# Orca0917/fine-grained-emotional-control-of-tts

Hardware: AMD Instinct MI355X
Metric: train mel-frames/sec at B=32, 80-bin mel; 1/2/4/8 MI355X (higher is better)
Workload: dtype bf16; 1 GPU; FastSpeech2 train step (fwd+loss+bwd+allreduce+AdamW), B=32/GPU, T_phon_max=200, T_mel_max=977, D=384 F=1536 6+6 FFT layers, 80 mels; global_batch=32, seq_len=977, parallelism=dp1

## Files before the change

fine-grained-emotional-control-of-tts_amd/csrc/gemm.hip:

```cpp
#include <type_traits>

#include "fs2_cdna.h"
#include "fs2_launch.h"

#include <cstdlib>
#include <cstring>

namespace {

#ifdef FS2_EXPERIMENTS
#define XFLAGS(p) ((p).g4_flags)
#else
#define XFLAGS(p) 0
#endif

constexpr int BM = 128, BN = 128, NT = 256;
constexpr int TILE_BYTES = 128 * 128;

struct GemmP {
  int M, N, K, kvalid, mvalid, nvalid;
  const char* A; long lda; const char* B; long ldb;
  int conv_mode, conv_t, conv_kw, conv_c, conv_p;
  int conv_dil;
  char* C; long ldc; int c_fp32; int c_conv_kw;
  const float* bias; int relu;
  const char* gate; long ldg;
  const float* row_scale;
  const char* residual; long ldr;
  const float* row_scale_post;
  int accumulate; int split_k; int k_per_split;
  long split_stride;
  int g4_flags;
  int batch_div;
  long sA1, sA2, sB1, sB2, sC1, sC2, sR1, sR2;
  int tiles_m, tiles_n;
  int vec_ok;
  int vec_align;
  int c_row_t, c_row_pad;
  int max_ctas;
  int a_bytes, b_bytes;
  int a_kw;
  const int32_t* k_eff;
};

__device__ __forceinline__ u32x4 add_bf16x8(u32x4 a, u32x4 b) {
  u32x4 r;
#pragma unroll
  for (int w = 0; w < 4; ++w) {
    float a0 = __builtin_bit_cast(float, a[w] << 16), a1 = __builtin_bit_cast(float, a[w] & 0xffff0000u);
    float b0 = __builtin_bit_cast(float, b[w] << 16), b1 = __builtin_bit_cast(float, b[w] & 0xffff0000u);
    bf16 r0 = (bf16)(a0 + b0), r1 = (bf16)(a1 + b1);
    r[w] = (unsigned)__builtin_bit_cast(unsigned short, r0) |
           ((unsigned)__builtin_bit_cast(unsigned short, r1) << 16);
  }
  return r;
}
__device__ __forceinline__ u32x4 add_f32x4(u32x4 a, u32x4 b) {
  const f32x4 fa = __builtin_bit_cast(f32x4, a), fb = __builtin_bit_cast(f32x4, b);
  return __builtin_bit_cast(u32x4, fa + fb);
}

__device__ __attribute__((noinline)) float epi_act_rare(float v, int act) {
  if (act == 2) return 0.5f * v * (1.f + erff(v * 0.70710678118654752f));
  if (act == 3) return v >= 0.f ? v : 0.1f * v;
  if (act == 4) return tanhf(v);
  return v;
}
__device__ __forceinline__ float epi_act(float v, int act) {
  if (act > 1) return epi_act_rare(v, act);
  return act ? fmaxf(v, 0.f) : v;
}

template <typename T>
struct Cfg {
  static constexpr int ES = sizeof(T);
  static constexpr int EPC = 16 / ES;
  static constexpr int BK = 8 * EPC;
};

__device__ __forceinline__ u32x4 ld16(const char* p) { return *(const u32x4*)p; }

template <typename T>
__device__ __forceinline__ void load_kmajor(u32x4 (&st)[4], const char* base, long ld, int row0,
                                            int nrows, int k0, int kend, const GemmP& p,
                                            int cmode, const int (&rb)[4], const int (&rt)[4]) {
  constexpr int ES = Cfg<T>::ES, EPC = Cfg<T>::EPC;
  const int tid = threadIdx.x;
  const int kc = tid & 7;
  const int k = k0 + kc * EPC;
#pragma unroll
  for (int i = 0; i < 4; ++i) {
    const int r = (tid >> 3) + 32 * i;
    const int row = row0 + r;
    u32x4 v = {0u, 0u, 0u, 0u};
    if (row < nrows && k < kend) {
      if (cmode == 0) {
        v = ld16(base + ((long)row * ld + k) * ES);
      } else {
        const int C = p.conv_c, T_ = p.conv_t, P = p.conv_p;
        const int j = k / C, c = k - j * C;
        const int b = rb[i], t = rt[i];
        if (cmode == 1) {
          const int ts = reflect_idx(t + (j - P) * p.conv_dil, T_);
          v = ld16(base + ((long)(b * T_ + ts) * ld + c) * ES);
        } else if (cmode == 5) {
          const int ts = t + (j - P) * p.conv_dil;
          if (ts >= 0 && ts < T_) v = ld16(base + ((long)(b * T_ + ts) * ld + c) * ES);
        } else if (cmode == 4) {
          const int ts = t - j;
          if (ts >= 0 && ts < T_) v = ld16(base + ((long)(b * T_ + ts) * ld + c) * ES);
        } else {
          const int t1 = t - j + P;
          if (t1 >= 0 && t1 < T_) v = ld16(base + ((long)(b * T_ + t1) * ld + c) * ES);
          const int t2 = P - j - t;
          if (t >= 1 && t2 >= 0 && t2 < T_) {
            u32x4 w = ld16(base + ((long)(b * T_ + t2) * ld + c) * ES);
            v = (ES == 2) ? add_bf16x8(v, w) : add_f32x4(v, w);
          }
          const int t3 = 2 * (T_ - 1) - t - j + P;
          if (t <= T_ - 2 && t3 >= 0 && t3 < T_ && t3 + j - P >= T_) {
            u32x4 w = ld16(base + ((long)(b * T_ + t3) * ld + c) * ES);
            v = (ES == 2) ? add_bf16x8(v, w) : add_f32x4(v, w);
          }
        }
      }
    }
// ... 153 lines not shown
  const int k1 = s * 32 + 8 * g + q, k2 = k1 + 4;
  const char* a1 = lds + k1 * ROWB + ((c ^ mn_swz<bf16>(k1)) << 4) + boff;
  const char* a2 = lds + k2 * ROWB + ((c ^ mn_swz<bf16>(k2)) << 4) + boff;
  s16x4 lo, hi;
  asm volatile("ds_read_b64_tr_b16 %0, %1" : "=v"(lo) : "v"(lds_off(a1)));
  asm volatile("ds_read_b64_tr_b16 %0, %1" : "=v"(hi) : "v"(lds_off(a2)));
  const s16x8 v = {lo[0], lo[1], lo[2], lo[3], hi[0], hi[1], hi[2], hi[3]};
  return __builtin_bit_cast(bf16x8, v);
}
__device__ __forceinline__ void mn_ready(bf16x8& f) { asm volatile("" : "+v"(f)); }

__device__ __forceinline__ float frag_f32_kmajor(const char* lds, int r0, int s, int lane) {
  const int r = r0 + (lane & 15);
  return *(const float*)(lds + r * 128 + ((s ^ (r & 7)) << 4) + (lane >> 4) * 4);
}
__device__ __forceinline__ float frag_f32_mnmajor(const char* lds, int r0, int s, int lane) {
  const int m = r0 + (lane & 15), k = s * 4 + (lane >> 4);
  return *(const float*)(lds + k * 512 + (((m >> 2) ^ mn_swz<float>(k)) << 4) + (m & 3) * 4);
}

template <typename T>
__device__ __forceinline__ void load8(float (&o)[8], const T* src, int nn) {
  if (nn == 8) {
    if constexpr (sizeof(T) == 2) {
      const u32x4 u = *(const u32x4*)src;
#pragma unroll
      for (int w = 0; w < 4; ++w) {
        o[2 * w] = __builtin_bit_cast(float, u[w] << 16);
        o[2 * w + 1] = __builtin_bit_cast(float, u[w] & 0xffff0000u);
      }
    } else {
      const f32x4 a = *(const f32x4*)src, b = *(const f32x4*)(src + 4);
      o[0] = a[0]; o[1] = a[1]; o[2] = a[2]; o[3] = a[3];
      o[4] = b[0]; o[5] = b[1]; o[6] = b[2]; o[7] = b[3];
    }
  } else {
    for (int e = 0; e < 8; ++e) o[e] = e < nn ? to_f(src[e]) : 0.f;
  }
}
template <typename T>
__device__ __forceinline__ void store8(T* dst, const float (&v)[8], int nn) {
  if (nn == 8) {
    if constexpr (sizeof(T) == 2) {
      u32x4 u;
#pragma unroll
      for (int w = 0; w < 4; ++w) {
        const bf16 a = (bf16)v[2 * w], b = (bf16)v[2 * w + 1];
        u[w] = (unsigned)__builtin_bit_cast(unsigned short, a) |
               ((unsigned)__builtin_bit_cast(unsigned short, b) << 16);
      }
      *(u32x4*)dst = u;
    } else {
      *(f32x4*)dst = f32x4{v[0], v[1], v[2], v[3]};
      *(f32x4*)(dst + 4) = f32x4{v[4], v[5], v[6], v[7]};
    }
  } else {
    for (int e = 0; e < nn; ++e) dst[e] = from_f<T>(v[e]);
  }
}

template <typename T, bool AK, bool BKM, bool GA, bool GB>
__global__ void __launch_bounds__(NT) gemm_kernel(GemmP p) {
  constexpr int ES = Cfg<T>::ES, BK = Cfg<T>::BK;
  __shared__ __attribute__((aligned(16))) char smem[2 * 2 * TILE_BYTES];

  const int tid = threadIdx.x, lane = tid & 63, wave = tid >> 6;
  const int wm = wave >> 1, wn = wave & 1;

  const int bid = blockIdx.x;
  const int tm = bid / p.tiles_n, tn = bid - tm * p.tiles_n;
  const int m0 = tm * BM, n0 = tn * BN;

  int z = 0, kbeg = 0, kend = p.K;
  if (p.split_k > 1) {
    kbeg = blockIdx.z * p.k_per_split;
    kend = min(p.K, kbeg + p.k_per_split);
  } else {
    z = blockIdx.z;
  }
  const long zb = z / p.batch_div, zh = z - zb * p.batch_div;
  const char* Ab = p.A + (zb * p.sA1 + zh * p.sA2) * ES;
  const char* Bb = p.B + (zb * p.sB1 + zh * p.sB2) * ES;
  const int kvalid = p.kvalid;

  int rb[4] = {0, 0, 0, 0}, rt[4] = {0, 0, 0, 0};
  const int amode = (p.conv_mode == 1 || p.conv_mode == 2 || p.conv_mode == 4 || p.conv_mode == 5) ? p.conv_mode : 0;
  if (AK && amode) {
#pragma unroll
    for (int i = 0; i < 4; ++i) {
      const int row = m0 + (GA ? (wave * 4 + i) * 8 + (lane >> 3) : (tid >> 3) + 32 * i);
      const int rpu = amode == 4 ? p.conv_t + 2 * p.conv_p : p.conv_t;
      rb[i] = row / rpu;
      rt[i] = row - rb[i] * rpu;
    }
  }
  const bool bconv3 = (p.conv_mode == 3);
  const int zero4[4] = {0, 0, 0, 0};

  f32x4 acc[4][4];
#pragma unroll
  for (int i = 0; i < 4; ++i)
#pragma unroll
    for (int j = 0; j < 4; ++j) acc[i][j] = f32x4{0.f, 0.f, 0.f, 0.f};

  u32x4 stA[4], stB[4];
  auto load_tiles = [&](int k0, int stage) {
    char* la = smem + stage * 2 * TILE_BYTES;
    char* lb = la + TILE_BYTES;
    const int wv = __builtin_amdgcn_readfirstlane(wave);
    if constexpr (GA) {
      if constexpr (AK) glds_kmajor(la, Ab, p.lda, m0, p.M, k0, kend, p, amode, rb, rt, wv, lane);
      else glds_mnmajor(la, Ab, p.lda, m0, p.M, k0, min(kend, kvalid), p, false, wv, lane);
    } else {
      if constexpr (AK) load_kmajor<T>(stA, Ab, p.lda, m0, p.M, k0, kend, p, amode, rb, rt);
      else load_mnmajor<T>(stA, Ab, p.lda, m0, p.M, k0, min(kend, kvalid), p, false);
    }
    if constexpr (GB) {
      if constexpr (BKM) glds_kmajor(lb, Bb, p.ldb, n0, p.N, k0, kend, p, 0, zero4, zero4, wv, lane);
      else glds_mnmajor(lb, Bb, p.ldb, n0, p.N, k0, min(kend, kvalid), p, bconv3, wv, lane);
    } else {
      if constexpr (BKM) load_kmajor<T>(stB, Bb, p.ldb, n0, p.N, k0, kend, p, 0, zero4, zero4);
      else load_mnmajor<T>(stB, Bb, p.ldb, n0, p.N, k0, min(kend, kvalid), p, bconv3);
    }
  };
  auto store_tiles = [&](int stage) {
    char* la = smem + stage * 2 * TILE_BYTES;
    char* lb = la + TILE_BYTES;
    if constexpr (!GA) { if constexpr (AK) store_kmajor<T>(la, stA); else store_mnmajor<T>(la, stA); }
    if constexpr (!GB) { if constexpr (BKM) store_kmajor<T>(lb, stB); else store_mnmajor<T>(lb, stB); }
  };

  const int nk = (kend > kbeg) ? (kend - kbeg + BK - 1) / BK : 0;
  if (nk > 0) {
    load_tiles(kbeg, 0);
    store_tiles(0);
  }
  __syncthreads();

  for (int kt = 0; kt < nk; ++kt) {
    const int stage = kt & 1;
    if (kt + 1 < nk) load_tiles(kbeg + (kt + 1) * BK, stage ^ 1);
    const char* la = smem + stage * 2 * TILE_BYTES;
    const char* lb = la + TILE_BYTES;
    if constexpr (ES == 2) {
#pragma unroll
      for (int s = 0; s < 2; ++s) {
        bf16x8 af[4], bfr[4];
#pragma unroll
        for (int i = 0; i < 4; ++i) {
          af[i] = AK ? frag_bf16_kmajor(la, wm * 64 + i * 16, s, lane)
                     : frag_bf16_mnmajor(la, wm * 64 + i * 16, s, lane);
          bfr[i] = BKM ? frag_bf16_kmajor(lb, wn * 64 + i * 16, s, lane)
                       : frag_bf16_mnmajor(lb, wn * 64 + i * 16, s, lane);
        }
#pragma unroll
        for (int i = 0; i < 4; ++i)
#pragma unroll
          for (int j = 0; j < 4; ++j)
            acc[i][j] = __builtin_amdgcn_mfma_f32_16x16x32_bf16(af[i], bfr[j], acc[i][j], 0, 0, 0);
      }
    } else {
#pragma unroll
      for (int s = 0; s < 8; ++s) {
        float af[4], bfr[4];
#pragma unroll
        for (int i = 0; i < 4; ++i) {
          af[i] = AK ? frag_f32_kmajor(la, wm * 64 + i * 16, s, lane)
                     : frag_f32_mnmajor(la, wm * 64 + i * 16, s, lane);
          bfr[i] = BKM ? frag_f32_kmajor(lb, wn * 64 + i * 16, s, lane)
                       : frag_f32_mnmajor(lb, wn * 64 + i * 16, s, lane);
        }
#pragma unroll
        for (int i = 0; i < 4; ++i)
#pragma unroll
          for (int j = 0; j < 4; ++j)
            acc[i][j] = __builtin_amdgcn_mfma_f32_16x16x4f32(af[i], bfr[j], acc[i][j], 0, 0, 0);
      }
    }
    if (kt + 1 < nk) store_tiles(stage ^ 1);
    __syncthreads();
  }

  const int OES = p.c_fp32 ? 4 : ES;
  char* Cb = p.C + (zb * p.sC1 + zh * p.sC2) * OES;
  if (p.split_stride > 0 && p.split_k > 1) Cb += (long)blockIdx.z * p.split_stride * OES;
  const char* Rb = p.residual ? p.residual + (zb * p.sR1 + zh * p.sR2) * ES : nullptr;
  const bool atomic = p.split_k > 1 && p.split_stride == 0;
  const int cc = p.c_conv_kw > 0 ? p.N / p.c_conv_kw : 0;
  if (!p.vec_ok) {
#pragma unroll
    for (int i = 0; i < 4; ++i) {
#pragma unroll
      for (int r = 0; r < 4; ++r) {
        const int m = m0 + wm * 64 + i * 16 + (lane >> 4) * 4 + r;
        if (m >= p.mvalid) continue;
        const float rs = p.row_scale ? p.row_scale[m] : 1.f;
        const float rs2 = p.row_scale_post ? p.row_scale_post[m] : 1.f;
#pragma unroll
        for (int j = 0; j < 4; ++j) {
          const int n = n0 + wn * 64 + j * 16 + (lane & 15);
          if (n >= p.nvalid) continue;
          float v = acc[i][j][r];
          if (p.bias) v += p.bias[n];
          v = epi_act(v, p.relu);
          if (p.gate) v = (to_f(((const T*)p.gate)[(long)m * p.ldg + n]) > 0.f) ? v : 0.f;
          v *= rs;
          if (Rb) v += to_f(((const T*)Rb)[(long)m * p.ldr + n]);
          v *= rs2;
          long col = n;
          if (cc > 0) { const int jj = n / cc; col = (long)(n - jj * cc) * p.c_conv_kw + jj; }
          const long off = (long)m * p.ldc + col;
          if (p.c_fp32) {
            float* Cf = (float*)Cb;
            if (atomic) atomicAdd(Cf + off, v);
            else if (p.accumulate) Cf[off] += v;
            else Cf[off] = v;
          } else {
            ((T*)Cb)[off] = from_f<T>(v);
          }
        }
      }
    }
    return;
  }
// ... 159 lines not shown
  const int n = n0 + c8;
  if (n >= p.nvalid) return;
  const int nn = min(8, p.nvalid - n);
  float bv[8] = {0.f, 0.f, 0.f, 0.f, 0.f, 0.f, 0.f, 0.f};
  if (p.bias) {
    if (nn == 8) {
      const f32x4 b0 = *(const f32x4*)(p.bias + n), b1 = *(const f32x4*)(p.bias + n + 4);
      bv[0] = b0[0]; bv[1] = b0[1]; bv[2] = b0[2]; bv[3] = b0[3];
      bv[4] = b1[0]; bv[5] = b1[1]; bv[6] = b1[2]; bv[7] = b1[3];
    } else {
      for (int e = 0; e < nn; ++e) bv[e] = p.bias[n + e];
    }
  }
#pragma unroll 2
  for (int pass = 0; pass < 8; ++pass) {
    const int row = (tid >> 4) + 32 * pass;
    const int m = m0 + row;
    if (m >= p.mvalid) continue;
    const int sw = cs_swz(row);
    const f32x4 lo = *(const f32x4*)&cs[row * 128 + (c8 ^ sw)];
    const f32x4 hi = *(const f32x4*)&cs[row * 128 + ((c8 + 4) ^ sw)];
    float v[8] = {lo[0], lo[1], lo[2], lo[3], hi[0], hi[1], hi[2], hi[3]};
    const float rs = p.row_scale ? p.row_scale[m] : 1.f;
    const float rs2 = p.row_scale_post ? p.row_scale_post[m] : 1.f;
    if (p.bias) {
#pragma unroll
      for (int e = 0; e < 8; ++e) v[e] += bv[e];
    }
    float g[8], rr[8];
    if (p.gate) load8<bf16>(g, (const bf16*)p.gate + (long)m * p.ldg + n, nn);
    if (Rb) load8<bf16>(rr, (const bf16*)Rb + (long)m * p.ldr + n, nn);
#pragma unroll
    for (int e = 0; e < 8; ++e) {
      float x = v[e];
      x = epi_act(x, p.relu);
      if (p.gate) x = (g[e] > 0.f) ? x : 0.f;
      x *= rs;
      if (Rb) x += rr[e];
      v[e] = x * rs2;
    }
    const long off = (long)m * p.ldc + n;
    if (p.c_fp32) {
      float* Cf = (float*)Cb + off;
      if (nn == 8) {
        f32x4 o0 = {v[0], v[1], v[2], v[3]}, o1 = {v[4], v[5], v[6], v[7]};
        if (p.accumulate) { o0 += *(const f32x4*)Cf; o1 += *(const f32x4*)(Cf + 4); }
        *(f32x4*)Cf = o0;
        *(f32x4*)(Cf + 4) = o1;
      } else {
        for (int e = 0; e < nn; ++e) Cf[e] = p.accumulate ? Cf[e] + v[e] : v[e];
      }
    } else {
      store8<bf16>((bf16*)Cb + off, v, nn);
    }
  }
}

template <bool AK, bool BKM, int CM, int B3>
__global__ void __launch_bounds__(BNT) gemm_big_kernel(GemmP p) {
  __shared__ __attribute__((aligned(16))) char smem[BIG_LDS];
  const int tid = threadIdx.x, lane = tid & 63;
  const int wave = __builtin_amdgcn_readfirstlane(tid >> 6);
  const int wm = wave >> 1, wn = wave & 1;
  const int nwg = p.tiles_m * p.tiles_n;
  const int orig = blockIdx.x;
  const int xcd = orig & 7, q = nwg >> 3, r8 = nwg & 7;
  const int bid = (xcd < r8 ? xcd * (q + 1) : r8 * (q + 1) + (xcd - r8) * q) + (orig >> 3);
  const int tm = bid / p.tiles_n, tn = bid - tm * p.tiles_n;
  const int m0 = tm * BBM, n0 = tn * 128;
  const int z = p.split_k > 1 ? 0 : blockIdx.z;
  const long zb = z / p.batch_div, zh = z - zb * p.batch_div;
  const char* Ab = p.A + (zb * p.sA1 + zh * p.sA2) * 2;
  const char* Bb = p.B + (zb * p.sB1 + zh * p.sB2) * 2;
  const int K = p.K;
  const int kva = min(K, p.kvalid);
  const int amode = CM >= 0 ? CM : ((p.conv_mode == 1 || p.conv_mode == 4 || p.conv_mode == 5) ? p.conv_mode : 0);
  const int nk_all = (K + 63) / 64;
  int kt0 = 0, kt1 = nk_all;
  if (p.split_k > 1) {
    const int kps = (nk_all + p.split_k - 1) / p.split_k;
    kt0 = blockIdx.z * kps;
    kt1 = min(nk_all, kt0 + kps);
  }
  const bool bconv3 = B3 >= 0 ? B3 == 1 : p.conv_mode == 3;
  const bool tap_uniform = CM > 0 ? true : (CM == 0 ? false : amode && (p.conv_c % 64) == 0);
  const int rpu = amode == 4 ? p.conv_t + 2 * p.conv_p : p.conv_t;

  const i32x4 rsA = make_rsrc(Ab), rsB = make_rsrc(Bb);
  int avo[4];
  int abt[4], at[4], alc[4];
  bool aval[4];
#pragma unroll
  for (int i = 0; i < 4; ++i) {
    if constexpr (AK) {
      const int r = (wave * 4 + i) * 8 + (lane >> 3);
      alc[i] = (lane & 7) ^ (r & 7);
      const int row = m0 + r;
      aval[i] = row < p.M;
      const int rr = aval[i] ? row : 0;
      const int b = amode ? rr / rpu : 0;
      abt[i] = b * p.conv_t;
      at[i] = rr - b * rpu;
      avo[i] = aval[i] ? (int)(((long)rr * p.lda + alc[i] * 8) * 2) : BUF_OOB;
    } else {
      const int kr = (wave * 4 + i) * 2 + (lane >> 5);
      alc[i] = (lane & 31) ^ mn_swz<bf16>(kr);
      at[i] = kr;
      const int mn = m0 + alc[i] * 8;
      aval[i] = mn < p.M;
      avo[i] = aval[i] ? (int)(((long)mn + (long)kr * p.lda) * 2) : BUF_OOB;
      abt[i] = 0;
    }
  }
  int a_tap = -1;
  int bvo[2];
  int blc[2], bkr[2], bb[2], bt[2];
  bool bval[2];
  int b_k = kt0 * 64;
#pragma unroll
  for (int i = 0; i < 2; ++i) {
    if constexpr (BKM) {
      const int r = (wave * 2 + i) * 8 + (lane >> 3);
      blc[i] = (lane & 7) ^ (r & 7);
      const int row = n0 + r;
      bval[i] = row < p.N;
      bvo[i] = bval[i] ? (int)(((long)row * p.ldb + blc[i] * 8) * 2) : BUF_OOB;
      bkr[i] = 0; bb[i] = 0; bt[i] = 0;
    } else {
      const int kr = (wave * 2 + i) * 4 + (lane >> 4);
      blc[i] = (lane & 15) ^ mn_swz<bf16>(kr);
      bkr[i] = kr;
      const int mn = n0 + blc[i] * 8;
      bval[i] = mn < p.N;
      int col = mn;
      if (bconv3 && bval[i]) { const int j = mn / p.conv_c; col = mn - j * p.conv_c; blc[i] = j; }
      else if (bconv3) blc[i] = 0;
      bvo[i] = bval[i] ? (int)(((long)col + (bconv3 ? 0L : (long)kr * p.ldb)) * 2) : BUF_OOB;
      const int k = b_k + kr;
      bb[i] = bconv3 ? k / p.conv_t : 0;
      bt[i] = bconv3 ? k - bb[i] * p.conv_t : 0;
    }
  }

  auto issue = [&](int kt, int stage) {
    const int k0 = kt * 64;
    char* la = smem + stage * BIG_STAGE;
    char* lb = la + BIG_A;
    if constexpr (AK) {
      if (amode && tap_uniform) {
        const int j = k0 / p.conv_c, c0 = k0 - j * p.conv_c;
        if (j != a_tap) {
          a_tap = j;
#pragma unroll
          for (int i = 0; i < 4; ++i) {
            int ts;
            bool ok = aval[i];
            if (amode == 1) {
              ts = reflect_idx(at[i] + (j - p.conv_p) * p.conv_dil, p.conv_t);
            } else {
              ts = amode == 5 ? at[i] + (j - p.conv_p) * p.conv_dil : at[i] - j;
              ok = ok && ts >= 0 && ts < p.conv_t;
            }
            avo[i] = ok ? (int)(((long)(abt[i] + ts) * p.lda + alc[i] * 8) * 2) : BUF_OOB;
          }
        }
        const bool kin = k0 + 64 <= K;
#pragma unroll
        for (int i = 0; i < 4; ++i) {
          const int vo = (kin || k0 + alc[i] * 8 < K) ? avo[i] : BUF_OOB;
          blds16(rsA, vo, c0 * 2, la + (wave * 4 + i) * 1024);
        }
      } else if (!amode) {
        const bool kin = k0 + 64 <= K;
#pragma unroll
        for (int i = 0; i < 4; ++i) {
          const int vo = (kin || k0 + alc[i] * 8 < K) ? avo[i] : BUF_OOB;
          blds16(rsA, vo, k0 * 2, la + (wave * 4 + i) * 1024);
        }
      } else {
#pragma unroll
        for (int i = 0; i < 4; ++i) {
          const int k = k0 + alc[i] * 8;
          bool ok = aval[i] && k < K;
          const int j = k / p.conv_c, c = k - j * p.conv_c;
          int ts;
          if (amode == 1) {
            ts = reflect_idx(at[i] + (j - p.conv_p) * p.conv_dil, p.conv_t);
          } else {
            ts = amode == 5 ? at[i] + (j - p.conv_p) * p.conv_dil : at[i] - j;
            ok = ok && ts >= 0 && ts < p.conv_t;
          }
          const int vo = ok ? (int)(((long)(abt[i] + ts) * p.lda + c) * 2) : BUF_OOB;
          blds16(rsA, vo, 0, la + (wave * 4 + i) * 1024);
        }
      }
    } else {
      const bool kin = k0 + 64 <= kva;
#pragma unroll
      for (int i = 0; i < 4; ++i) {
        const int vo = (kin || k0 + at[i] < kva) ? avo[i] : BUF_OOB;
        blds16(rsA, vo, (int)((long)k0 * p.lda * 2), la + (wave * 4 + i) * 1024);
      }
    }
    if constexpr (BKM) {
      const bool kin = k0 + 64 <= K;
#pragma unroll
      for (int i = 0; i < 2; ++i) {
        const int vo = (kin || k0 + blc[i] * 8 < K) ? bvo[i] : BUF_OOB;
        blds16(rsB, vo, k0 * 2, lb + (wave * 2 + i) * 1024);
      }
    } else if (!bconv3) {
      const bool kin = k0 + 64 <= kva;
#pragma unroll
      for (int i = 0; i < 2; ++i) {
        const int vo = (kin || k0 + bkr[i] < kva) ? bvo[i] : BUF_OOB;
        blds16(rsB, vo, (int)((long)k0 * p.ldb * 2), lb + (wave * 2 + i) * 1024);
      }
    } else {
      const int dk = k0 - b_k;
      b_k = k0;
#pragma unroll
      for (int i = 0; i < 2; ++i) {
        int t = bt[i] + dk, b = bb[i];
        while (t >= p.conv_t) { t -= p.conv_t; ++b; }
        bt[i] = t; bb[i] = b;
        int ts = t + blc[i] - p.conv_p;
        ts = ts < 0 ? -ts : (ts >= p.conv_t ? 2 * (p.conv_t - 1) - ts : ts);
        const bool ok = bval[i] && k0 + bkr[i] < kva;
        const int vo = ok ? bvo[i] + (int)(((long)b * p.conv_t + ts) * p.ldb * 2) : BUF_OOB;
        blds16(rsB, vo, 0, lb + (wave * 2 + i) * 1024);
      }
    }
  };

  f32x4 acc[4][4];
#pragma unroll
  for (int i = 0; i < 4; ++i)
#pragma unroll
    for (int j = 0; j < 4; ++j) acc[i][j] = f32x4{0.f, 0.f, 0.f, 0.f};

  const int nk = kt1 - kt0;
  if (nk > 0) issue(kt0, 0);
  if (nk > 1) issue(kt0 + 1, 1);
  for (int it = 0; it < nk; ++it) {
    if (it + 1 < nk) asm volatile("s_waitcnt vmcnt(6)" ::: "memory");
    else asm volatile("s_waitcnt vmcnt(0)" ::: "memory");
    asm volatile("s_waitcnt lgkmcnt(0)" ::: "memory");
    __builtin_amdgcn_s_barrier();
    __builtin_amdgcn_sched_barrier(0);
    if (it + 2 < nk) issue(kt0 + it + 2, (it + 2) % 3);
    const char* la = smem + (it % 3) * BIG_STAGE;
    const char* lb = la + BIG_A;
    bf16x8 af[2][4], bfr[2][4];
#pragma unroll
    for (int s = 0; s < 2; ++s)
#pragma unroll
      for (int i = 0; i < 4; ++i) {
        af[s][i] = AK ? frag_bf16_kmajor(la, wm * 64 + i * 16, s, lane)
                      : frag_bf16_mnmajor_asm<512>(la, wm * 64 + i * 16, s, lane);
        bfr[s][i] = BKM ? frag_bf16_kmajor(lb, wn * 64 + i * 16, s, lane)
                        : frag_bf16_mnmajor_asm<256>(lb, wn * 64 + i * 16, s, lane);
      }
    if constexpr (!AK || !BKM) {
      asm volatile("s_waitcnt lgkmcnt(0)" ::: "memory");
#pragma unroll
      for (int s = 0; s < 2; ++s)
#pragma unroll
        for (int i = 0; i < 4; ++i) {
          if constexpr (!AK) mn_ready(af[s][i]);
          if constexpr (!BKM) mn_ready(bfr[s][i]);
        }
    }
#pragma unroll
    for (int s = 0; s < 2; ++s)
#pragma unroll
      for (int i = 0; i < 4; ++i)
#pragma unroll
        for (int j = 0; j < 4; ++j)
          acc[i][j] = __builtin_amdgcn_mfma_f32_16x16x32_bf16(bfr[s][j], af[s][i], acc[i][j], 0, 0, 0);
    if constexpr (AK && BKM) {
      __builtin_amdgcn_sched_group_barrier(0x100, 16, 0);
      __builtin_amdgcn_sched_group_barrier(0x008, 32, 0);
    }
  }
  asm volatile("s_waitcnt vmcnt(0) lgkmcnt(0)" ::: "memory");

  char* Cb = p.C + (zb * p.sC1 + zh * p.sC2) * (p.c_fp32 ? 4 : 2);
  if (p.split_stride > 0 && p.split_k > 1) Cb += (long)blockIdx.z * p.split_stride * 4;
  const char* Rb = p.residual ? p.residual + (zb * p.sR1 + zh * p.sR2) * 2 : nullptr;
  if (p.vec_ok && !(XFLAGS(p) & 64)) {
    epilogue_direct(p, &acc[0][0], m0 + wm * 64, n0 + wn * 64, Cb, Rb, lane);
    return;
  }
  __syncthreads();
  float* cs = (float*)smem;
#pragma unroll
  for (int i = 0; i < 4; ++i)
#pragma unroll
    for (int j = 0; j < 4; ++j)
#pragma unroll
      for (int r = 0; r < 4; ++r) {
        const int row = wm * 64 + i * 16 + (lane & 15);
        const int col = wn * 64 + j * 16 + (lane >> 4) * 4 + r;
        cs[row * 128 + (col ^ cs_swz(row))] = acc[i][j][r];
      }
  __syncthreads();
  epilogue_256x128(p, cs, m0, n0, Cb, Rb, tid);
}

constexpr int G4_NT = 512;
constexpr int G4_REG = 16384;
constexpr int G4_SLOT = 4 * G4_REG;
constexpr int G4_LDS = 2 * G4_SLOT;

__device__ __forceinline__ int g4_fsw(int row) { return (0x78 >> (2 * ((row >> 2) & 3))) & 3; }

__device__ __forceinline__ bf16x8 g4_frag_k(const char* rg, int row, int g) {
  return *(const bf16x8*)(rg + row * 64 + ((g ^ g4_fsw(row)) << 4));
}

template <bool AK, bool BKM, int CM, int B3>
__global__ void __launch_bounds__(G4_NT, 1) gemm256_kernel(GemmP p) {
  __shared__ __attribute__((aligned(16))) char smem[G4_LDS];
  const int tid = threadIdx.x, lane = tid & 63;
  const int wave = __builtin_amdgcn_readfirstlane(tid >> 6);
  const int wr = wave >> 2, wc = wave & 3;
  const int nwg = p.tiles_m * p.tiles_n;
  const int orig = blockIdx.x;
  const int xcd = orig & 7, q8 = nwg >> 3, r8 = nwg & 7;
  const int bid = (xcd < r8 ? xcd * (q8 + 1) : r8 * (q8 + 1) + (xcd - r8) * q8) + (orig >> 3);
  const int tm = bid / p.tiles_n, tn = bid - tm * p.tiles_n;
  const int m0 = tm * 256, n0 = tn * 256;
  const int z = p.split_k > 1 ? 0 : blockIdx.z;
  const long zb = z / p.batch_div, zh = z - zb * p.batch_div;
  const char* Ab = p.A + (zb * p.sA1 + zh * p.sA2) * 2;
  const char* Bb = p.B + (zb * p.sB1 + zh * p.sB2) * 2;
  const int K = p.K;
  const int kva = min(K, p.kvalid);
  const int amode = CM >= 0 ? CM : ((p.conv_mode == 1 || p.conv_mode == 4 || p.conv_mode == 5) ? p.conv_mode : 0);
  const int nk_all = (K + 63) / 64;
  int kt0 = 0, kt1 = nk_all;
  if (p.split_k > 1) {
    const int kps = (nk_all + p.split_k - 1) / p.split_k;
    kt0 = blockIdx.z * kps;
    kt1 = min(nk_all, kt0 + kps);
  }
  const bool bconv3 = B3 >= 0 ? B3 == 1 : p.conv_mode == 3;
  const bool tap_uniform = CM > 0 ? true : (CM == 0 ? false : amode && (p.conv_c % 32) == 0);
  const int rpu = amode == 4 ? p.conv_t + 2 * p.conv_p : p.conv_t;

  const i32x4 rsA = make_rsrc(Ab), rsB = make_rsrc(Bb);
  int avo[2];
  int abt[2], at[2], ac[2];
  bool aval[2];
#pragma unroll
  for (int i = 0; i < 2; ++i) {
    const int piece = wave * 2 + i;
    if constexpr (AK) {
      const int r = piece * 16 + (lane >> 2);
      ac[i] = (lane & 3) ^ g4_fsw(r);
      const int row = m0 + r;
      aval[i] = row < p.M;
      const int rr = aval[i] ? row : 0;
      const int b = amode ? rr / rpu : 0;
      abt[i] = b * p.conv_t;
      at[i] = rr - b * rpu;
      avo[i] = aval[i] ? (int)(((long)rr * p.lda + ac[i] * 8) * 2) : BUF_OOB;
      if (XFLAGS(p) & 128) {
        const int r2 = m0 + piece * 16 + (lane >> 3) + 8 * i;
        avo[i] = r2 < p.M ? (int)(((long)r2 * p.lda + (lane & 7) * 8) * 2) : BUF_OOB;
      }
    } else {
      const int kr = piece * 2 + (lane >> 5);
      ac[i] = (lane & 31) ^ mn_swz<bf16>(kr);
      at[i] = kr;
      const int mn = m0 + ac[i] * 8;
      aval[i] = mn < p.M;
      avo[i] = aval[i] ? (int)(((long)mn + (long)kr * p.lda) * 2) : BUF_OOB;
      abt[i] = 0;
    }
  }
  int a_tap = -1;
  int bvo[2];
  int bc[2], bkr[2], bb[2], bt[2];
  bool bval[2];
  int b_k = kt0 * 64;
#pragma unroll
  for (int i = 0; i < 2; ++i) {
    const int piece = wave * 2 + i;
    if constexpr (BKM) {
      const int r = piece * 16 + (lane >> 2);
      bc[i] = (lane & 3) ^ g4_fsw(r);
      const int row = n0 + r;
      bval[i] = row < p.N;
      bvo[i] = bval[i] ? (int)(((long)row * p.ldb + bc[i] * 8) * 2) : BUF_OOB;
      if (XFLAGS(p) & 128) {
        const int r2 = n0 + piece * 16 + (lane >> 3) + 8 * i;
        bvo[i] = r2 < p.N ? (int)(((long)r2 * p.ldb + (lane & 7) * 8) * 2) : BUF_OOB;
      }
      bkr[i] = 0; bb[i] = 0; bt[i] = 0;
    } else {
      const int kr = piece * 2 + (lane >> 5);
      const int lc = (lane & 31) ^ mn_swz<bf16>(kr);
      bkr[i] = kr;
      const int mn = n0 + lc * 8;
      bval[i] = mn < p.N;
      int col = mn;
      bc[i] = 0;
      if (bconv3 && bval[i]) { const int j = mn / p.conv_c; col = mn - j * p.conv_c; bc[i] = j; }
      bvo[i] = bval[i] ? (int)(((long)col + (bconv3 ? 0L : (long)kr * p.ldb)) * 2) : BUF_OOB;
      const int k = b_k + kr;
      bb[i] = bconv3 ? k / p.conv_t : 0;
      bt[i] = bconv3 ? k - bb[i] * p.conv_t : 0;
    }
  }

  auto issueA = [&](char* dst, int k0) {
    if constexpr (AK) {
      if (amode && tap_uniform) {
        const int j = k0 / p.conv_c;
        const int c0 = k0 - j * p.conv_c;
        if (j != a_tap) {
          a_tap = j;
#pragma unroll
          for (int i = 0; i < 2; ++i) {
            int ts;
            bool ok = aval[i];
            if (amode == 1) {
              ts = reflect_idx(at[i] + (j - p.conv_p) * p.conv_dil, p.conv_t);
            } else {
              ts = amode == 5 ? at[i] + (j - p.conv_p) * p.conv_dil : at[i] - j;
              ok = ok && ts >= 0 && ts < p.conv_t;
            }
            avo[i] = ok ? (int)(((long)(abt[i] + ts) * p.lda + ac[i] * 8) * 2) : BUF_OOB;
          }
        }
        const bool kin = k0 + 32 <= K;
#pragma unroll
        for (int i = 0; i < 2; ++i) {
          const int vo = (kin || k0 + ac[i] * 8 < K) ? avo[i] : BUF_OOB;
          blds16(rsA, vo, c0 * 2, dst + (wave * 2 + i) * 1024);
        }
      } else if (!amode) {
        const bool kin = k0 + 32 <= K;
#pragma unroll
        for (int i = 0; i < 2; ++i) {
          const int vo = (kin || k0 + ac[i] * 8 < K) ? avo[i] : BUF_OOB;
          blds16(rsA, vo, ((XFLAGS(p) & 128) ? (k0 & ~63) : k0) * 2, dst + (wave * 2 + i) * 1024);
        }
      } else {
#pragma unroll
        for (int i = 0; i < 2; ++i) {
          const int k = k0 + ac[i] * 8;
          bool ok = aval[i] && k < K;
          const int j = k / p.conv_c, c = k - j * p.conv_c;
          int ts;
          if (amode == 1) {
            ts = reflect_idx(at[i] + (j - p.conv_p) * p.conv_dil, p.conv_t);
          } else {
            ts = amode == 5 ? at[i] + (j - p.conv_p) * p.conv_dil : at[i] - j;
            ok = ok && ts >= 0 && ts < p.conv_t;
          }
          const int vo = ok ? (int)(((long)(abt[i] + ts) * p.lda + c) * 2) : BUF_OOB;
          blds16(rsA, vo, 0, dst + (wave * 2 + i) * 1024);
        }
      }
    } else {
      const bool kin = k0 + 32 <= kva;
#pragma unroll
      for (int i = 0; i < 2; ++i) {
        const int vo = (kin || k0 + at[i] < kva) ? avo[i] : BUF_OOB;
        blds16(rsA, vo, (int)((long)k0 * p.lda * 2), dst + (wave * 2 + i) * 1024);
      }
    }
  };
  auto issueB = [&](char* dst, int k0) {
    if constexpr (BKM) {
      const bool kin = k0 + 32 <= K;
#pragma unroll
      for (int i = 0; i < 2; ++i) {
        const int vo = (kin || k0 + bc[i] * 8 < K) ? bvo[i] : BUF_OOB;
        blds16(rsB, vo, ((XFLAGS(p) & 128) ? (k0 & ~63) : k0) * 2, dst + (wave * 2 + i) * 1024);
      }
    } else if (!bconv3) {
      const bool kin = k0 + 32 <= kva;
#pragma unroll
      for (int i = 0; i < 2; ++i) {
        const int vo = (kin || k0 + bkr[i] < kva) ? bvo[i] : BUF_OOB;
        blds16(rsB, vo, (int)((long)k0 * p.ldb * 2), dst + (wave * 2 + i) * 1024);
      }
    } else {
      const int dk = k0 - b_k;
      b_k = k0;
#pragma unroll
      for (int i = 0; i < 2; ++i) {
        int t = bt[i] + dk, b = bb[i];
        while (t >= p.conv_t) { t -= p.conv_t; ++b; }
        bt[i] = t; bb[i] = b;
        int ts = t + bc[i] - p.conv_p;
        ts = ts < 0 ? -ts : (ts >= p.conv_t ? 2 * (p.conv_t - 1) - ts : ts);
        const bool ok = bval[i] && k0 + bkr[i] < kva;
        const int vo = ok ? bvo[i] + (int)(((long)b * p.conv_t + ts) * p.ldb * 2) : BUF_OOB;
        blds16(rsB, vo, 0, dst + (wave * 2 + i) * 1024);
      }
    }
  };
  auto issue = [&](int it, int reg) {
    const int k0 = (kt0 + it) * 64 + (reg >> 1) * 32;
    char* dst = smem + (it & 1) * G4_SLOT + reg * G4_REG;
    if ((reg & 1) == 0) issueA(dst, k0);
    else issueB(dst, k0);
  };

  f32x4 acc[8][4];
#pragma unroll
  for (int i = 0; i < 8; ++i)
#pragma unroll
    for (int j = 0; j < 4; ++j) acc[i][j] = f32x4{0.f, 0.f, 0.f, 0.f};

  const int nk = kt1 - kt0;
  if (nk > 0) {
    issue(0, 1); issue(0, 0); issue(0, 3); issue(0, 2);
  }
  if (nk > 1) {
    issue(1, 1); issue(1, 0);
    asm volatile("s_waitcnt vmcnt(8)" ::: "memory");
  } else {
    asm volatile("s_waitcnt vmcnt(4)" ::: "memory");
  }
  __builtin_amdgcn_s_barrier();
  const bool stag = !(XFLAGS(p) & 1);
  const bool prio = !(XFLAGS(p) & 2);
  const bool nowait = XFLAGS(p) & 4;
  const bool noissue = XFLAGS(p) & 8;
  const int grp = stag ? wr : 1;
  if (stag && wr == 1) __builtin_amdgcn_s_barrier();
  __builtin_amdgcn_sched_barrier(0);

  bf16x8 af[4], bfr[4];
  for (int it = 0; it < nk; ++it) {
    const bool more = it + 1 < nk;
#pragma unroll
    for (int ph = 0; ph < 4; ++ph) {
      const int s = ph >> 1, mq = ph & 1;
      const char* rA = smem + (it & 1) * G4_SLOT + (2 * s) * G4_REG;
      const char* rB = rA + G4_REG;
      if (mq == 0) {
#pragma unroll
        for (int j = 0; j < 4; ++j)
          bfr[j] = BKM ? g4_frag_k(rB, wc * 64 + j * 16 + (lane & 15), lane >> 4)
                       : frag_bf16_mnmajor_asm<512>(rB, wc * 64 + j * 16, 0, lane);
      }
#pragma unroll
      for (int i = 0; i < 4; ++i)
        af[i] = AK ? g4_frag_k(rA, wr * 128 + mq * 64 + i * 16 + (lane & 15), lane >> 4)
                   : frag_bf16_mnmajor_asm<512>(rA, wr * 128 + mq * 64 + i * 16, 0, lane);
      const bool iss = !noissue && (ph < 2 ? more : it + 2 < nk);
      if (iss) issue(ph < 2 ? it + 1 : it + 2, 3 - ph);
      if (grp == 1 && (ph & 1) && !nowait && !noissue) {
        if (iss) {
          asm volatile("s_waitcnt vmcnt(8)" ::: "memory");
        } else if (ph == 3 && more) asm volatile("s_waitcnt vmcnt(4)" ::: "memory");
        else asm volatile("s_waitcnt vmcnt(0)" ::: "memory");
      }
      __builtin_amdgcn_s_barrier();
      __builtin_amdgcn_sched_barrier(0);
      asm volatile("s_waitcnt lgkmcnt(0)" ::: "memory");
      if constexpr (!AK) {
#pragma unroll
        for (int i = 0; i < 4; ++i) mn_ready(af[i]);
      }
      if constexpr (!BKM) {
#pragma unroll
        for (int j = 0; j < 4; ++j) mn_ready(bfr[j]);
      }
      if (prio) __builtin_amdgcn_s_setprio(1);
#pragma unroll
      for (int i = 0; i < 4; ++i) {
#pragma unroll
        for (int j = 0; j < 4; ++j)
          acc[mq * 4 + i][j] =
              __builtin_amdgcn_mfma_f32_16x16x32_bf16(af[i], bfr[j], acc[mq * 4 + i][j], 0, 0, 0);
      }
      if (prio) __builtin_amdgcn_s_setprio(0);
      if (grp == 0 && (ph & 1) && !nowait && !noissue) {
        if (ph == 1 ? more : it + 2 < nk) asm volatile("s_waitcnt vmcnt(8)" ::: "memory");
        else if (ph == 3 && more) asm volatile("s_waitcnt vmcnt(4)" ::: "memory");
        else asm volatile("s_waitcnt vmcnt(0)" ::: "memory");
      }
      __builtin_amdgcn_s_barrier();
      __builtin_amdgcn_sched_barrier(0);
    }
  }
  if (stag && wr == 0) __builtin_amdgcn_s_barrier();
  asm volatile("s_waitcnt vmcnt(0) lgkmcnt(0)" ::: "memory");

  __syncthreads();

  char* Cb = p.C + (zb * p.sC1 + zh * p.sC2) * (p.c_fp32 ? 4 : 2);
  if (p.split_stride > 0 && p.split_k > 1) Cb += (long)blockIdx.z * p.split_stride * 4;
  const char* Rb = p.residual ? p.residual + (zb * p.sR1 + zh * p.sR2) * 2 : nullptr;
  float* cs = (float*)smem;
#pragma unroll
  for (int h = 0; h < 2; ++h) {
    if ((wc >> 1) == h) {
#pragma unroll
      for (int i = 0; i < 8; ++i)
#pragma unroll
        for (int j = 0; j < 4; ++j)
#pragma unroll
          for (int r = 0; r < 4; ++r) {
            const int row = wr * 128 + i * 16 + (lane >> 4) * 4 + r;
            const int col = (wc & 1) * 64 + j * 16 + (lane & 15);
            cs[row * 128 + (col ^ cs_swz(row))] = acc[i][j][r];
          }
    }
    __syncthreads();
    if (n0 + h * 128 < p.nvalid) epilogue_256x128(p, cs, m0, n0 + h * 128, Cb, Rb, tid);
    __syncthreads();
  }
}

constexpr int G4R_REG = 16384;
__device__ __forceinline__ int g4r_sw(int r) { return (r >> 1) & 7; }
__device__ __forceinline__ bf16x8 g4r_frag(const char* rg, int row, int chunk) {
  return *(const bf16x8*)(rg + row * 128 + ((chunk ^ g4r_sw(row)) << 4));
}

template <int CM, bool TR = false, int WN = 64>
__global__ void __launch_bounds__(G4_NT, 1) gemm256r_kernel(GemmP p) {
  static_assert(WN == 64 || (WN == 48 && TR), "the 192-wide tile has only the direct epilogue");
  constexpr int NJ = WN / 16, BR = 2 * WN;
  __shared__ __attribute__((aligned(16))) char smem[G4_LDS];
  const int tid = threadIdx.x, lane = tid & 63;
  const int wave = __builtin_amdgcn_readfirstlane(tid >> 6);
  const int wr = wave >> 2, wc = wave & 3;
  const int nwg = p.tiles_m * p.tiles_n;
  const int orig = blockIdx.x;
  const int xcd = orig & 7, q8 = nwg >> 3, r8 = nwg & 7;
  const int bid = (xcd < r8 ? xcd * (q8 + 1) : r8 * (q8 + 1) + (xcd - r8) * q8) + (orig >> 3);
  const int tm = bid / p.tiles_n, tn = bid - tm * p.tiles_n;
  const int m0 = tm * 256, n0 = tn * (4 * WN);
  const int z = p.split_k > 1 ? 0 : blockIdx.z;
  const long zb = z / p.batch_div, zh = z - zb * p.batch_div;
  const char* Ab = p.A + (zb * p.sA1 + zh * p.sA2) * 2;
  const char* Bb = p.B + (zb * p.sB1 + zh * p.sB2) * 2;
  const int K = p.K;
  const int nk_all = (K + 63) / 64;
  int kt0 = 0, kt1 = nk_all;
  if (p.split_k > 1) {
    const int kps = (nk_all + p.split_k - 1) / p.split_k;
    kt0 = blockIdx.z * kps;
    kt1 = min(nk_all, kt0 + kps);
  }
  const int rpu = CM == 4 ? p.conv_t + 2 * p.conv_p : p.conv_t;

  const i32x4 rsA = make_rsrc(Ab), rsB = make_rsrc(Bb);
  int lc[2];
  int avo[4], at[4], abt[4];
  bool aval[4];
  int bvo[4];
#pragma unroll
  for (int i = 0; i < 2; ++i) {
    const int rho = (2 * wave + i) * 8 + (lane >> 3);
    lc[i] = (lane & 7) ^ g4r_sw(rho);
#pragma unroll
    for (int q = 0; q < 2; ++q) {
      const int idx = q * 2 + i;
      const int row = m0 + (rho < 64 ? rho : rho + 64) + q * 64;
      aval[idx] = row < p.M;
      const int rr = aval[idx] ? row : 0;
      const int b = CM ? rr / rpu : 0;
      abt[idx] = b * p.conv_t;
      at[idx] = rr - b * rpu;
      avo[idx] = aval[idx] ? (int)(((long)rr * p.lda + lc[i] * 8) * 2) : BUF_OOB;
// ... 1057 lines not shown
            const bool ok = rowok && n < p.nvalid && !nost;
            llvm_raw_buffer_store_v2i32(i32x2{(int)a[0], (int)a[1]}, rsC,
                                        ok ? ((m * (int)p.ldc + n) * 2) : BUF_OOB, 0, 0);
          }
        }
      }
      __builtin_amdgcn_s_barrier();
      __builtin_amdgcn_sched_barrier(0);
    };
    phase(std::integral_constant<int, 0>{});
    phase(std::integral_constant<int, 1>{});
    phase(std::integral_constant<int, 2>{});
    phase(std::integral_constant<int, 3>{});
    if (++kt == nk) { kt = 0; ++t; }
  }
  if (wr == 0) __builtin_amdgcn_s_barrier();
  asm volatile("s_waitcnt vmcnt(0)" ::: "memory");
}


struct GemmKernel { const char* name; void (*fn)(GemmP); int block; };
#define FS2_K(block, ...) {#__VA_ARGS__, __VA_ARGS__, block}
#define FS2_K128(T, GA, GB)                                        \
  FS2_K(NT, gemm_kernel<T, true, true, GA, GB>), FS2_K(NT, gemm_kernel<T, true, false, GA, GB>), \
  FS2_K(NT, gemm_kernel<T, false, true, GA, GB>), FS2_K(NT, gemm_kernel<T, false, false, GA, GB>)
#define FS2_KTILE(K, nt)                                           \
  FS2_K(nt, K<true, true, 1, 0>), FS2_K(nt, K<true, true, 4, 0>),                             \
  FS2_K(nt, K<true, true, 5, 0>), FS2_K(nt, K<true, true, -1, -1>),                           \
  FS2_K(nt, K<false, false, 0, 1>), FS2_K(nt, K<false, false, 0, 0>),                         \
  FS2_K(nt, K<false, false, -1, -1>), FS2_K(nt, K<true, false, -1, -1>),                      \
  FS2_K(nt, K<false, true, -1, -1>)
const GemmKernel KERNELS[] = {
    FS2_K(W4_NT, gemm_w4b_kernel<true, 6>), FS2_K(W4_NT, gemm_w4b_kernel<false, 6>),
    FS2_K(W4_NT, gemm_w4b_kernel<true, 8>), FS2_K(W4_NT, gemm_w4b_kernel<false, 8>),
    FS2_K(BNT, gemm_ps_kernel<0, 64, 0, 1>),
    FS2_K(NT, gemm_kernel<bf16, true, true, false, true>),
    FS2_K(NT, gemm_kernel<bf16, true, false, false, true>),
    FS2_K128(bf16, true, true),
    FS2_K(BNT, gemm_ps_kernel<0, 48, 1, 0>),
    FS2_K(BNT, gemm_ps_kernel<0, 48, 0, 0>), FS2_K(BNT, gemm_ps_kernel<4, 48, 0, 0>),
    FS2_K(BNT, gemm_ps_kernel<0, 64, 0, 0>), FS2_K(BNT, gemm_ps_kernel<4, 64, 0, 0>),
    FS2_K(BNT, gemm_pk_kernel<4, 4>), FS2_K(BNT, gemm_pk_kernel<2, 4>), FS2_K(BNT, gemm_pk_kernel<2, 2>),
    FS2_K(G4_NT, gemm256r_kernel<0, true, 64>), FS2_K(G4_NT, gemm256r_kernel<1, true, 64>),
    FS2_K(G4_NT, gemm256r_kernel<0, false, 64>), FS2_K(G4_NT, gemm256r_kernel<1, false, 64>),
    FS2_K(G4_NT, gemm256r_kernel<4, false, 64>), FS2_K(G4_NT, gemm256r_kernel<5, false, 64>),
    FS2_KTILE(gemm256_kernel, G4_NT),
    FS2_K(BNT, gemm_big_kernel<true, true, 0, 0>), FS2_KTILE(gemm_big_kernel, BNT),
    FS2_K128(float, false, false),
};
enum { K_W4B = 0, K_PS6 = 4, K_128C2 = 5, K_128 = 7, K_PS = 11, K_PK = 16, K_256R = 19, K_256 = 25,
       K_BIG = 34, K_F32 = 44, K_COUNT = 48 };
static_assert(sizeof(KERNELS) / sizeof(KERNELS[0]) == K_COUNT, "kernel table out of step");

struct GemmArgs { GemmP p; int dtype, ak, bk, batch; };

struct GemmPlan { int kernel; dim3 grid; GemmP p; };

int conv_variant(const GemmP& q, int granule) {
  if (q.conv_mode == 0 || q.conv_mode == 3) return 0;
  if ((q.conv_mode == 1 || q.conv_mode == 4 || q.conv_mode == 5) && q.conv_c % granule == 0)
    return q.conv_mode;
  return -1;
}

int tile_variant(int ak, int bk, int cm, int conv_mode) {
  if (ak && bk) return cm == 0 ? 0 : cm == 1 ? 1 : cm == 4 ? 2 : cm == 5 ? 3 : 4;
  if (!ak && !bk) return conv_mode == 3 ? 5 : conv_mode == 0 ? 6 : 7;
  return ak ? 8 : 9;
}

int validate(const fs2_gemm_desc* d, GemmArgs& a) {
  if (!d || d->M < 0 || d->N < 0 || d->K < 0) return FS2_EINVAL;
  if (d->M == 0 || d->N == 0) return 1;
  const int es = d->dtype == FS2_BF16 ? 2 : 4;
  const int epc = 16 / es;
  const int bk = 8 * epc;
  a = GemmArgs{};
  GemmP& p = a.p;
  p.M = d->M; p.N = d->N; p.K = d->K;
  p.kvalid = d->kvalid > 0 ? d->kvalid : d->K;
  p.mvalid = d->mvalid > 0 ? min(d->mvalid, d->M) : d->M;
  p.nvalid = d->nvalid > 0 ? min(d->nvalid, d->N) : d->N;
  p.A = (const char*)d->A; p.lda = d->lda; p.B = (const char*)d->B; p.ldb = d->ldb;
  p.conv_mode = d->conv_mode; p.conv_t = d->conv_t; p.conv_kw = d->conv_kw; p.conv_c = d->conv_c;
  p.conv_p = d->conv_kw > 0 ? (d->conv_kw - 1) / 2 : 0;
  p.conv_dil = d->conv_dil > 1 ? d->conv_dil : 1;
  p.C = (char*)d->C; p.ldc = d->ldc; p.c_fp32 = d->c_fp32; p.c_conv_kw = d->c_conv_kw;
  p.bias = d->bias; p.relu = d->relu;
  p.gate = (const char*)d->gate; p.ldg = d->ldg;
  p.row_scale = d->row_scale;
  p.residual = (const char*)d->residual; p.ldr = d->ldr;
  p.row_scale_post = d->row_scale_post;
  p.accumulate = d->accumulate;
  p.split_k = d->split_k > 1 ? d->split_k : 1;
  p.split_stride = d->split_stride > 0 ? d->split_stride : 0;
  p.batch_div = d->batch_div > 0 ? d->batch_div : 1;
  p.sA1 = d->sA1; p.sA2 = d->sA2; p.sB1 = d->sB1; p.sB2 = d->sB2;
  p.sC1 = d->sC1; p.sC2 = d->sC2; p.sR1 = d->sR1; p.sR2 = d->sR2;
  p.tiles_m = (p.M + BM - 1) / BM;
  p.tiles_n = (p.N + BN - 1) / BN;
  const int batch = d->batch > 1 ? d->batch : 1;
  p.c_row_t = d->c_row_t > 0 ? d->c_row_t : 0;
  p.c_row_pad = p.c_row_t ? d->c_row_pad : 0;
  p.max_ctas = d->max_ctas > 0 && d->max_ctas < 256 ? max(8, d->max_ctas / 8 * 8) : 256;
  p.a_kw = d->a_kw > 0 ? d->a_kw : 0;
  p.k_eff = d->k_eff;
  if (p.k_eff && (d->conv_mode != 6 || p.K < 128)) return FS2_EINVAL;
  if (p.a_kw && (d->dtype != FS2_BF16 || !d->a_kmajor || !d->b_kmajor || d->conv_mode ||
                 batch > 1 || p.split_k > 1 || p.lda % 64 ||
                 (long)p.a_kw * p.lda != p.K))
    return FS2_EINVAL;
  if (p.c_row_t && (d->dtype != FS2_BF16 || !d->a_kmajor || !d->b_kmajor ||
                    p.conv_mode || batch > 1 || p.split_k > 1 || p.accumulate || p.c_conv_kw))
    return FS2_EINVAL;

  if (!p.A || !p.B || !p.C) return FS2_EINVAL;
  if (p.K % epc) return FS2_EINVAL;
  if (!aligned16(p.A) || !aligned16(p.B)) return FS2_EALIGN;
  if ((p.lda % epc) || (p.ldb % epc)) return FS2_EALIGN;
  if ((batch > 1) && ((p.sA1 | p.sA2 | p.sB1 | p.sB2) % epc)) return FS2_EALIGN;
  if (!d->a_kmajor && (p.M % epc)) return FS2_EINVAL;
  if (!d->b_kmajor && (p.N % epc)) return FS2_EINVAL;
  if (p.conv_mode) {
    if (p.conv_t <= 0 || p.conv_kw <= 0 || p.conv_c <= 0 || (p.conv_c % epc)) return FS2_EINVAL;
    if (p.conv_dil > 1 && p.conv_mode != 1 && p.conv_mode != 5) return FS2_EINVAL;
    if ((p.conv_mode == 1 || p.conv_mode == 2 || p.conv_mode == 3) && p.conv_p * p.conv_dil >= p.conv_t)
      return FS2_EINVAL;
    if ((p.conv_mode == 1 || p.conv_mode == 2 || p.conv_mode == 5) && (!d->a_kmajor || p.K != p.conv_kw * p.conv_c))
      return FS2_EINVAL;
    if ((p.conv_mode == 1 || p.conv_mode == 2 || p.conv_mode == 5) && (p.M % p.conv_t)) return FS2_EINVAL;
    if (p.conv_mode == 4 && (p.M % (p.conv_t + 2 * p.conv_p))) return FS2_EINVAL;
    if (p.conv_mode == 4 && !d->a_kmajor) return FS2_EINVAL;
    if (p.conv_mode == 4 && p.K != p.conv_kw * p.conv_c) return FS2_EINVAL;
    if (p.conv_mode == 3 && (d->b_kmajor || p.N != p.conv_kw * p.conv_c)) return FS2_EINVAL;
    if (p.conv_mode == 6) {
      if (d->dtype != FS2_BF16 || !d->a_kmajor || !d->b_kmajor || !p.c_fp32 ||
          p.N != p.conv_kw * p.conv_c || (p.K % 64) || p.bias || p.gate || p.residual ||
          p.row_scale || p.row_scale_post || p.relu || p.c_conv_kw || batch > 1 || p.accumulate)
        return FS2_EINVAL;
      if (p.split_k > 1 && (p.split_stride <= 0 || (p.K % (64 * p.split_k)))) return FS2_EINVAL;
      const long lim = 0x7fffffffL;
      if ((long)p.M * p.lda * 2 >= lim || ((long)p.conv_c * p.ldb + 2 * BT_GUARD) * 2 >= lim ||
          (long)p.split_k * (p.split_stride + (long)p.mvalid * p.ldc) * 4 >= lim)
        return FS2_EINVAL;
    }
  }
  if (p.c_conv_kw > 0 && (p.N % p.c_conv_kw)) return FS2_EINVAL;
  if (p.split_k > 1) {
    if (!p.c_fp32 || batch > 1) return FS2_EINVAL;
    if (p.split_stride > 0 && (p.accumulate || p.split_stride < (long)(p.mvalid - 1) * p.ldc + p.nvalid))
      return FS2_EINVAL;
    const int nkt = (p.K + bk - 1) / bk;
    const int kps = (nkt + p.split_k - 1) / p.split_k;
    p.k_per_split = kps * bk;
    p.split_k = (nkt + kps - 1) / kps;
  }
  if (p.accumulate && !p.c_fp32) return FS2_EINVAL;
  const int ov = 16 / (p.c_fp32 ? 4 : es);
  bool v = p.c_conv_kw == 0 && aligned16(p.C) && (p.ldc % 8) == 0;
  if (batch > 1) v = v && ((p.sC1 | p.sC2) % ov) == 0 && ((p.sR1 | p.sR2) % epc) == 0;
  if (p.bias) v = v && aligned16(p.bias);
  if (p.gate) v = v && aligned16(p.gate) && (p.ldg % 8) == 0;
  if (p.residual) v = v && aligned16(p.residual) && (p.ldr % 8) == 0;
  v = v && (p.nvalid % 4) == 0;
  p.vec_align = v;
  p.vec_ok = v && (p.split_k <= 1 || p.split_stride > 0);
  if (p.split_stride > 0 && p.split_k <= 1) p.split_stride = 0;
  a.dtype = d->dtype; a.ak = d->a_kmajor != 0; a.bk = d->b_kmajor != 0; a.batch = batch;
  return 0;
}

int plan_gemm(const GemmArgs& a, GemmPlan& pl) {
  const GemmP& p = a.p;
  const int ak = a.ak, bk = a.bk;
  const int gz = p.split_k > 1 ? p.split_k : a.batch;
  pl.p = p;
  pl.grid = dim3(p.tiles_m * p.tiles_n, 1, gz);
  GemmP& q = pl.p;
  const int major = 3 - (2 * ak + bk);
  if (a.dtype == FS2_F32) { pl.kernel = K_F32 + major; return 0; }
  if (a.dtype != FS2_BF16) return FS2_EINVAL;
  const int k128 = p.conv_mode == 2 ? K_128C2 + major : K_128 + major;
  const int tiles_big = ((p.M + BBM - 1) / BBM) * p.tiles_n;
  const int batch = p.split_k > 1 ? 1 : gz;
  const bool wgrad = p.split_stride == 0 && p.c_fp32 && (p.accumulate || p.split_k > 1) &&
                     batch == 1 && !p.gate &&
                     !p.residual && !p.bias && !p.row_scale && !p.row_scale_post && !p.relu &&
                     p.c_conv_kw == 0 && p.vec_align;
  auto own_split = [&](int tgt, int tiles) {
    return wgrad ? max(1, min((tgt + tiles - 1) / tiles, (p.K + 63) / 64 / 8)) : 1;
  };
// ... 188 lines not shown
```

fine-grained-emotional-control-of-tts_amd/csrc/norm.hip:

```cpp
#include <cstdlib>
#include <algorithm>
#include "fs2_launch.h"

namespace {

constexpr int MAXJ = 16;

template <bool DPP>
__device__ __forceinline__ float wsum(float v) {
  if constexpr (DPP) return wave_sum_dpp(v);
  else return wave_sum(v);
}

struct LnFwdP {
  const char* x; long ldx; const char* r; long ldr; float p_r; uint32_t salt_r;
  char* s_out; const float* gamma; const float* beta; float eps; int do_tanh;
  float p_o; uint32_t salt_o; const float* row_mask; const char* post_add; long ldp;
  char* y; long ldy; float* mean; float* rstd; int M, D; uint32_t seed;
  char* img; int img_t, img_p;
};

template <typename T>
__global__ void __launch_bounds__(256) ln_fwd_kernel(LnFwdP p) {
  const int lane = threadIdx.x & 63;
// ... 813 lines not shown
      const int jl = jr + 32 * pass, j = j0 + jl;
      u32x4 v = {0u, 0u, 0u, 0u};
      if (j < jend && c0 + ch * 8 < C) {
        int b, t, te = T;
        if (offs) {
          b = b0;
          int s = s0, e = e4[0];
#pragma unroll
          for (int i = 0; i < 3; ++i)
            if (j >= e4[i]) { ++b; s = e4[i]; e = e4[i + 1]; }
          while (j >= e && b + 1 < B) { ++b; s = e; e = offs[b + 1]; }
          t = j - s - P;
          te = min(T, e - s - 2 * P);
        } else {
          b = j / Tp;
          t = j - b * Tp - P;
        }
        bool ok = true;
        if (reflect) t = min(max(reflect_idx(t, T), 0), T - 1);
        else ok = t >= 0 && t < te;
        if (ok) v = *(const u32x4*)(X + ((long)b * T + t) * ldx + c0 + ch * 8);
      }
      *(u32x4*)(tile + jl * PITCH + ch * 16) = v;
    }
  }
  __syncthreads();
  {
    const int cr = tid >> 3, jc = tid & 7;
#pragma unroll
    for (int pass = 0; pass < 2; ++pass) {
      const int cl = cr + 32 * pass, c = c0 + cl;
      const int j = j0 + jc * 8;
      const unsigned short* col = (const unsigned short*)(tile + jc * 8 * PITCH) + cl;
      u32x4 w;
#pragma unroll
      for (int e = 0; e < 4; ++e)
        w[e] = (unsigned)col[(2 * e) * (PITCH / 2)] | ((unsigned)col[(2 * e + 1) * (PITCH / 2)] << 16);
      if (part && prow >= 0) {
        float s = 0.f;
#pragma unroll
        for (int e = 0; e < 4; ++e)
          s += bf16_bits_to_f((unsigned short)(w[e] & 0xffffu)) + bf16_bits_to_f((unsigned short)(w[e] >> 16));
        s += __shfl_xor(s, 1, 64);
        s += __shfl_xor(s, 2, 64);
        s += __shfl_xor(s, 4, 64);
        if (jc == 0 && c < C) part[(long)prow * C + c] = s;
      }
      if (c >= C || j >= ncols) continue;
      *(u32x4*)(out + (long)c * ldo + j) = w;
    }
  }
}

__global__ void __launch_bounds__(256) zero_f32_kernel(float* x, long n) {
  const long i = (long)blockIdx.x * 256 + threadIdx.x;
  if (i < n) x[i] = 0.f;
}

__global__ void __launch_bounds__(64) grad_tail_bounds_kernel(const int64_t* len, int B, int T,
                                                              int halo, int P, int32_t* end,
                                                              int32_t* offs, int noffs) {
  const int lane = threadIdx.x;
  int carry = 0;
  if (offs && lane == 0) offs[0] = 0;
  for (int b0 = 0; b0 < B; b0 += 64) {
    const int b = b0 + lane;
    int w = 0;
    if (b < B) {
      const long v = (long)len[b] + halo;
      const int e = (int)(v < 0 ? 0 : (v > T ? T : v));
      w = fs2_km_width(b, e, T, P);
      if (end) end[b] = e;
    }
#pragma unroll
    for (int d = 1; d < 64; d <<= 1) {
      const int o = __shfl_up(w, d, 64);
      if (lane >= d) w += o;
    }
    if (offs && b < B) offs[b + 1] = carry + w;
    carry += __shfl(w, 63, 64);
  }
  if (offs)
    for (int i = B + 1 + lane; i < noffs; i += 64) offs[i] = 0x7fffffff;
}

__global__ void __launch_bounds__(256) pad_rows_kernel(const bf16* X, long ldx, int B, int T,
                                                       int C8, int P, int reflect, bf16* out,
                                                       long ldo, unsigned n8) {
  const unsigned idx = blockIdx.x * 256u + threadIdx.x;
  if (idx >= n8) return;
  const unsigned r = idx / (unsigned)C8;
  const int c = (int)(idx - r * (unsigned)C8) * 8;
  const unsigned L = (unsigned)(T + 2 * P);
  const unsigned b = r / L;
  const int i = (int)(r - b * L) - P;
  u32x4 v = {0u, 0u, 0u, 0u};
  if ((int)b < B) {
    const int t = reflect ? reflect_idx(i, T) : i;
    if (t >= 0 && t < T) v = *(const u32x4*)(X + ((long)b * T + t) * ldx + c);
  }
  *(u32x4*)(out + (long)r * ldo + c) = v;
}

int colsum_blocks(int M) { return min(512, max(1, (M + 63) / 64)); }

}

extern "C" int64_t fs2_ln_workspace_floats(int M, int D) { return 3L * ln_blocks(M) * D; }
extern "C" int64_t fs2_colsum_workspace_floats(int M, int N) { return (int64_t)colsum_blocks(M) * N; }

extern "C" int fs2_ln_fwd(const void* x, int64_t ldx, const void* r, int64_t ldr, float p_r,
                          uint32_t salt_r, void* s_out, const float* gamma, const float* beta,
                          float eps, int do_tanh, float p_o, uint32_t salt_o,
                          const float* row_mask, const void* post_add, int64_t ldp, void* y,
                          int64_t ldy, float* mean, float* rstd, int M, int D, int dtype,
                          uint32_t seed, void* img, int img_t, int img_p, void* stream) {
  if (M <= 0) return 0;
  if (D <= 0 || D > 64 * MAXJ || !x || !y || !gamma || !beta || !mean || !rstd) return FS2_EINVAL;
  if (img && (dtype != FS2_BF16 || img_t <= 0 || M % img_t || img_p < 0 || img_p >= img_t ||
              (D % 8) || !aligned16(img)))
    return FS2_EINVAL;
  LnFwdP p{(const char*)x, ldx, (const char*)r, ldr, p_r, salt_r, (char*)s_out, gamma, beta,
           eps, do_tanh, p_o, salt_o, row_mask, (const char*)post_add, ldp, (char*)y, ldy, mean,
           rstd, M, D, seed, nullptr, img_t, img_p};
  bool img_done = false;
  dim3 grid((M + 3) / 4);
  hipStream_t s = (hipStream_t)stream;
  const int V = vec_elems(dtype);
  const int nch = (D / V + 63) / 64;
  const bool vec = (D % V) == 0 && nch <= 4 && aligned16(x) && (ldx % V) == 0 && aligned16(y) &&
                   (ldy % V) == 0 && aligned16(gamma) && aligned16(beta) && (!r || (aligned16(r) && ldr % V == 0)) &&
                   (!s_out || aligned16(s_out)) && (!post_add || (aligned16(post_add) && ldp % V == 0));
  if (dtype == FS2_BF16) {
    if (!vec) hipLaunchKernelGGL(ln_fwd_kernel<bf16>, grid, dim3(256), 0, s, p);
    else if (nch == 1) {
      p.img = (char*)img;
      img_done = true;
      hipLaunchKernelGGL((ln_fwd_rows_kernel<2, true>), dim3((M + 7) / 8), dim3(256), 0, s, p);
    }
    else if (nch == 2) hipLaunchKernelGGL((ln_fwd_vec_kernel<bf16, 2>), grid, dim3(256), 0, s, p);
    else hipLaunchKernelGGL((ln_fwd_vec_kernel<bf16, 4>), grid, dim3(256), 0, s, p);
  } else if (dtype == FS2_F32) {
    if (!vec) hipLaunchKernelGGL(ln_fwd_kernel<float>, grid, dim3(256), 0, s, p);
    else if (nch == 1) hipLaunchKernelGGL((ln_fwd_vec_kernel<float, 1>), grid, dim3(256), 0, s, p);
    else if (nch == 2) hipLaunchKernelGGL((ln_fwd_vec_kernel<float, 2>), grid, dim3(256), 0, s, p);
    else hipLaunchKernelGGL((ln_fwd_vec_kernel<float, 4>), grid, dim3(256), 0, s, p);
  } else {
    return FS2_EINVAL;
  }
  FS2_CHECK_LAUNCH();
  if (img && !img_done)
    return fs2_pad_rows(y, ldy, M / img_t, img_t, D, img_p, 1, 0, img, D, dtype, stream);
  return 0;
}

extern "C" int fs2_ln_bwd(const void* dy, int64_t lddy, const void* s, int64_t lds,
                          const float* mean, const float* rstd, const float* gamma,
                          const float* beta, int do_tanh, float p_o, uint32_t salt_o,
                          const float* row_mask, int relu_gate_in, void* ds, int64_t ldds,
                          void* dr, float p_r, uint32_t salt_r, float* dgamma, float* dbeta,
                          float* dcol, int M, int D, int dtype, uint32_t seed, float* workspace,
                          void* stream) {
  if (M <= 0) return 0;
  if (D <= 0 || D > 64 * MAXJ || !dy || !s || !ds || !gamma || !beta || !mean || !rstd)
    return FS2_EINVAL;
  if ((dgamma || dbeta) && (!dgamma || !dbeta)) return FS2_EINVAL;
// ... 97 lines not shown
  if (nsplit > 1 && (split_stride < (long)B * (T + 2 * P) * C || (split_stride % 4)))
    return FS2_EINVAL;
  const dim3 g((unsigned)((n / 4 + 255) / 256)), b(256);
  hipStream_t s = (hipStream_t)stream;
  const bool v8 = dtype == FS2_BF16 && C % 8 == 0 && aligned16(out) && ldo % 8 == 0 &&
                  (!residual || (aligned16(residual) && ldr % 8 == 0)) && aligned16(Xpad) &&
                  (nsplit == 1 || split_stride % 4 == 0) && n / 8 < (1L << 31);
  if (v8) {
    const unsigned n8 = (unsigned)(n / 8);
    hipLaunchKernelGGL(conv_fold8_kernel, dim3((n8 + 255) / 256), b, 0, s, Xpad, nsplit,
                       (long)split_stride, T, P, C / 8, (bf16*)out, (long)ldo,
                       (const bf16*)residual, (long)ldr, row_scale, row_scale_post, n8);
    FS2_CHECK_LAUNCH();
    return 0;
  }
  return dispatch_dtype(dtype, [&](auto t) {
    using U = decltype(t);
    hipLaunchKernelGGL(conv_fold_kernel<U>, g, b, 0, s, Xpad, nsplit, (long)split_stride, T, P, C,
                       (U*)out, (long)ldo, (const U*)residual, (long)ldr, row_scale,
                       row_scale_post, n);
  });
}

FS2_SEED_SETTER(fs2_seed_base_norm)

static int pad_transpose_impl(const void* X, int64_t ldx, int B, int T, int C, int P,
                              int reflect, void* out, int64_t ldo, int ncols, float* colsum,
                              float* workspace, const int32_t* offs, int ksplit, int dtype,
                              void* stream) {
  if (B <= 0 || T <= 0 || C <= 0) return 0;
  if (dtype != FS2_BF16 || !X || !out || P < 0 || (reflect && P >= T)) return FS2_EINVAL;
  if ((C % 8) || (ldx % 8) || (ldo % 8) || (ncols % 8) || ncols < (long)B * (T + 2 * P) ||
      ldo < ncols || !aligned16(X) || !aligned16(out))
    return FS2_EALIGN;
  if (colsum && (reflect || !workspace)) return FS2_EINVAL;
  if (offs && (ksplit < 1 || (ncols % (64 * ksplit)) || ncols < 128)) return FS2_EINVAL;
  dim3 grid((ncols + TJ - 1) / TJ, (C + TC - 1) / TC);
  hipStream_t s = (hipStream_t)stream;
  if (offs && colsum) {
    const long n = (long)grid.x * C;
    hipLaunchKernelGGL(zero_f32_kernel, dim3((unsigned)((n + 255) / 256)), dim3(256), 0, s,
                       workspace, n);
    FS2_CHECK_LAUNCH();
  }
  hipLaunchKernelGGL(pad_transpose_kernel, grid, dim3(256), 0, s, (const bf16*)X, (long)ldx, B, T,
                     C, P, reflect, (bf16*)out, (long)ldo, ncols, colsum ? workspace : nullptr,
                     offs, ksplit);
  FS2_CHECK_LAUNCH();
  if (colsum) {
    launch_reduce_parts(s, workspace, (int)grid.x, C, 1, colsum, nullptr, nullptr, 1);
    FS2_CHECK_LAUNCH();
  }
  return 0;
}

extern "C" int fs2_pad_transpose(const void* X, int64_t ldx, int B, int T, int C, int P,
                                 int reflect, void* out, int64_t ldo, int ncols, float* colsum,
                                 float* workspace, int dtype, void* stream) {
  return pad_transpose_impl(X, ldx, B, T, C, P, reflect, out, ldo, ncols, colsum, workspace,
                            nullptr, 1, dtype, stream);
}

extern "C" int fs2_pad_transpose_bounded(const void* X, int64_t ldx, int B, int T, int C, int P,
                                         int reflect, void* out, int64_t ldo, int ncols,
                                         float* colsum, float* workspace, const int32_t* offs,
                                         int ksplit, int dtype, void* stream) {
  if (!offs) return FS2_EINVAL;
  return pad_transpose_impl(X, ldx, B, T, C, P, reflect, out, ldo, ncols, colsum, workspace, offs,
                            ksplit, dtype, stream);
}

extern "C" int fs2_grad_tail_bounds(const int64_t* len, int B, int T, int halo, int P,
                                    int32_t* end, int32_t* offs, int noffs, void* stream) {
  if (B <= 0) return 0;
  if (!len || T <= 0 || halo < 0 || P < 0 || (!end && !offs)) return FS2_EINVAL;
  if (offs && (noffs < (B + 1 + 15) / 16 * 16 + 16 || (long)B * (T + 2L * P) >= 0x7fffffffL))
    return FS2_EINVAL;
  hipLaunchKernelGGL(grad_tail_bounds_kernel, dim3(1), dim3(64), 0, (hipStream_t)stream, len, B, T,
                     halo, P, end, offs, noffs);
  FS2_CHECK_LAUNCH();
  return 0;
}

extern "C" int fs2_pad_rows(const void* X, int64_t ldx, int B, int T, int C, int P, int reflect,
                            int tail, void* out, int64_t ldo, int dtype, void* stream) {
  if (B <= 0 || T <= 0 || C <= 0) return 0;
  if (dtype != FS2_BF16 || !X || !out || P < 0 || tail < 0 || (reflect && P >= T))
    return FS2_EINVAL;
  if ((C % 8) || (ldx % 8) || (ldo % 8) || ldo < C || ldx < C || !aligned16(X) || !aligned16(out))
    return FS2_EALIGN;
  const long rows = (long)B * (T + 2 * P) + tail;
  const long n8 = rows * (C / 8);
  if (n8 >= 0x7fffffffL || rows * ldo >= 0x7fffffffL) return FS2_EINVAL;
  hipLaunchKernelGGL(pad_rows_kernel, dim3((unsigned)((n8 + 255) / 256)), dim3(256), 0,
                     (hipStream_t)stream, (const bf16*)X, (long)ldx, B, T, C / 8, P, reflect,
                     (bf16*)out, (long)ldo, (unsigned)n8);
  FS2_CHECK_LAUNCH();
  return 0;
}
```

fine-grained-emotional-control-of-tts_amd/fastspeech2/_native.py:

```python

import ctypes
import os

import torch

_HERE = os.path.dirname(os.path.abspath(__file__))
LIB_PATH = os.environ.get("FS2_HIP_LIB", os.path.join(_HERE, "libfs2_hip.so"))
EXPERIMENTS = os.path.basename(LIB_PATH).startswith("libfs2_hip_exp")


def exp_flag(name, default=False):
    if not EXPERIMENTS:
        return default
    v = os.environ.get(name)
    return default if v is None else v not in ("", "0")


def exp_int(name, default):
    if not EXPERIMENTS:
        return default
    v = os.environ.get(name)
    return default if v is None else int(v)

F32 = 0
# ... 2 lines not shown

class NativeLibraryError(RuntimeError):
    pass


class GemmDesc(ctypes.Structure):
    _fields_ = [
        ("M", ctypes.c_int), ("N", ctypes.c_int), ("K", ctypes.c_int), ("kvalid", ctypes.c_int),
        ("mvalid", ctypes.c_int), ("nvalid", ctypes.c_int), ("dtype", ctypes.c_int),
        ("A", ctypes.c_void_p), ("lda", ctypes.c_int64), ("a_kmajor", ctypes.c_int),
        ("B", ctypes.c_void_p), ("ldb", ctypes.c_int64), ("b_kmajor", ctypes.c_int),
        ("conv_mode", ctypes.c_int), ("conv_t", ctypes.c_int), ("conv_kw", ctypes.c_int),
        ("conv_c", ctypes.c_int),
        ("C", ctypes.c_void_p), ("ldc", ctypes.c_int64), ("c_fp32", ctypes.c_int),
        ("c_conv_kw", ctypes.c_int),
        ("bias", ctypes.c_void_p), ("relu", ctypes.c_int),
        ("gate", ctypes.c_void_p), ("ldg", ctypes.c_int64),
        ("row_scale", ctypes.c_void_p),
        ("residual", ctypes.c_void_p), ("ldr", ctypes.c_int64),
        ("row_scale_post", ctypes.c_void_p),
        ("accumulate", ctypes.c_int), ("split_k", ctypes.c_int),
        ("split_stride", ctypes.c_int64),
        ("batch", ctypes.c_int), ("batch_div", ctypes.c_int),
        ("sA1", ctypes.c_int64), ("sA2", ctypes.c_int64), ("sB1", ctypes.c_int64),
        ("sB2", ctypes.c_int64), ("sC1", ctypes.c_int64), ("sC2", ctypes.c_int64),
        ("sR1", ctypes.c_int64), ("sR2", ctypes.c_int64), ("conv_dil", ctypes.c_int),
        ("c_row_t", ctypes.c_int), ("c_row_pad", ctypes.c_int), ("max_ctas", ctypes.c_int),
        ("a_kw", ctypes.c_int), ("k_eff", ctypes.c_void_p),
    ]


class GemmPlanInfo(ctypes.Structure):
    _fields_ = [
        ("kernel", ctypes.c_char * 64), ("grid", ctypes.c_int * 3), ("block", ctypes.c_int),
        ("tiles_m", ctypes.c_int), ("tiles_n", ctypes.c_int), ("split_k", ctypes.c_int),
        ("k_per_split", ctypes.c_int), ("vec_ok", ctypes.c_int), ("accumulate", ctypes.c_int),
    ]


class LossDesc(ctypes.Structure):
    _fields_ = [
        ("B", ctypes.c_int), ("Tm", ctypes.c_int), ("Tp", ctypes.c_int), ("NM", ctypes.c_int),
        ("dtype", ctypes.c_int),
        ("mel_out", ctypes.c_void_p), ("postnet_out", ctypes.c_void_p),
        ("log_dur", ctypes.c_void_p), ("pitch_pred", ctypes.c_void_p),
        ("energy_pred", ctypes.c_void_p),
        ("mel_tgt", ctypes.c_void_p), ("dur_tgt", ctypes.c_void_p),
        ("pitch_avg", ctypes.c_void_p), ("energy_avg", ctypes.c_void_p),
        ("mel_len", ctypes.c_void_p), ("phon_len", ctypes.c_void_p),
        ("w_ssim", ctypes.c_float), ("w_mel", ctypes.c_float), ("w_post", ctypes.c_float),
        ("w_dur", ctypes.c_float), ("w_pitch", ctypes.c_float), ("w_energy", ctypes.c_float),
        ("loss_out", ctypes.c_void_p),
        ("d_mel_out", ctypes.c_void_p), ("d_postnet_out", ctypes.c_void_p),
        ("d_log_dur", ctypes.c_void_p), ("d_pitch", ctypes.c_void_p), ("d_energy", ctypes.c_void_p),
        ("workspace", ctypes.c_void_p),
    ]


class WPrepDesc(ctypes.Structure):
    _fields_ = [
        ("W", ctypes.c_void_p), ("Wf", ctypes.c_void_p), ("Wb", ctypes.c_void_p),
        ("O", ctypes.c_int), ("C", ctypes.c_int), ("KW", ctypes.c_int), ("w_okc", ctypes.c_int),
        ("ldf", ctypes.c_int), ("ldb", ctypes.c_int), ("tile0", ctypes.c_int),
        ("tiles_k", ctypes.c_int),
    ]


P = ctypes.c_void_p
I = ctypes.c_int
I64 = ctypes.c_int64
U32 = ctypes.c_uint32
Fl = ctypes.c_float

SIGNATURES = {
    "fs2_gemm": (I, [ctypes.POINTER(GemmDesc), P]),
    "fs2_gemm_plan": (I, [ctypes.POINTER(GemmDesc), ctypes.POINTER(GemmPlanInfo)]),
    "fs2_colsum": (I, [P, I64, I, I, I, P, I, P, P]),
    "fs2_conv_fold": (I, [P, I, I64, I, I, I, I, P, I64, P, I64, P, P, I, P]),
    "fs2_colsum_workspace_floats": (I64, [I, I]),
    "fs2_sum_slices": (I, [P, I, I64, I64, P, I, P]),
    "fs2_pad_transpose": (I, [P, I64, I, I, I, I, I, P, I64, I, P, P, I, P]),
    "fs2_pad_transpose_bounded": (I, [P, I64, I, I, I, I, I, P, I64, I, P, P, P, I, I, P]),
    "fs2_grad_tail_bounds": (I, [P, I, I, I, I, P, P, I, P]),
    "fs2_pad_rows": (I, [P, I64, I, I, I, I, I, I, P, I64, I, P]),
    "fs2_ln_fwd": (I, [P, I64, P, I64, Fl, U32, P, P, P, Fl, I, Fl, U32, P, P, I64, P, I64, P, P,
                       I, I, I, U32, P, I, I, P]),
    "fs2_ln_bwd": (I, [P, I64, P, I64, P, P, P, P, I, Fl, U32, P, I, P, I64, P, Fl, U32, P, P, P,
                       I, I, I, U32, P, P]),
    "fs2_ln_workspace_floats": (I64, [I, I]),
    "fs2_attn_supported": (I, [I, I, I]),
    "fs2_attn_fwd": (I, [P, I64, P, I, I, I, I, I, Fl, Fl, U32, U32, P, I64, P, I, P]),
    "fs2_attn_bwd": (I, [P, I64, P, I, P, I64, P, I64, P, I, I, I, I, Fl, Fl, U32, U32, P, I64,
                         P, I, P]),
    "fs2_attn_bwd_bounded": (I, [P, I64, P, I, P, I64, P, I64, P, I, I, I, I, Fl, Fl, U32, U32, P,
                                 I64, P, P, I, P]),
    "fs2_attn_workspace_floats": (I64, [I, I, I]),
    "fs2_softmax_fwd": (I, [P, P, I, I, I, I, I, I, Fl, Fl, U32, U32, P, P, I, P]),
    "fs2_softmax_bwd": (I, [P, P, I, I, I, I, I, Fl, Fl, U32, U32, P, I, P]),
    "fs2_embed_fwd": (I, [P, P, P, I, I, I, I, P, P, I, P]),
    "fs2_embed_bwd": (I, [P, P, P, I, I, I, P, P, I, P]),
    "fs2_embed_bwd_workspace_floats": (I64, [I, I]),
    "fs2_keypad_from_tokens": (I, [P, I, I, P, P]),
    "fs2_keypad_from_lengths": (I, [P, I, I, P, P, P]),
    "fs2_concat_fwd": (I, [P, P, P, P, I, I, I, I, P, I, I, P]),
    "fs2_concat_bwd_spk": (I, [P, I, P, I, I, I, I, P, I, P, P]),
    "fs2_mask_rows": (I, [P, I64, P, I, I, I, P]),
    "fs2_add3_mask_rows": (I, [P, P, P, I64, P, I, I, I, P]),
    "fs2_rowdot_fwd": (I, [P, I64, P, P, Fl, I, I, P, I, P]),
    "fs2_rowdot_bwd": (I, [P, P, I64, P, Fl, I, I, P, P, P, I, P, P]),
    "fs2_avg_over_durations": (I, [P, I, P, I, I, P, P, P]),
    "fs2_avg_workspace_floats": (I64, [I, I]),
    "fs2_embed1d_fwd": (I, [P, P, P, P, I, I, I, I, P, I, P]),
    "fs2_embed1d_bwd": (I, [P, P, I, I, I, I, P, P, I, P, P]),
    "fs2_lr_index": (I, [P, I, Fl, I, I, I, P, P, P, P]),
    "fs2_lr_gather": (I, [P, P, P, I, I, I, I, P, P, I, P]),
    "fs2_lr_scatter": (I, [P, P, P, I, I, I, I, P, I, P]),
    "fs2_loss_fwd_bwd": (I, [ctypes.POINTER(LossDesc), P]),
    "fs2_loss_workspace_floats": (I64, [I, I, I]),
    "fs2_loss_fwd": (I, [ctypes.POINTER(LossDesc), P]),
    "fs2_loss_fwd_workspace_floats": (I64, [I, I, I]),
    "fs2_adamw": (I, [P, P, P, P, I64, Fl, Fl, Fl, Fl, Fl, Fl, Fl, Fl, P]),
    "fs2_weight_prep": (I, [P, I, I, I, I, P, I, P, I, I, P]),
    "fs2_weight_prep_batched": (I, [P, I, I, I, P]),
    "fs2_adamw_prep": (I, [P, I, I, P, I, I, P, P, P, P, Fl, Fl, Fl, Fl, Fl, Fl, Fl, Fl, I, P]),
    "fs2_intensity_input": (I, [P, I, I, I, I, P, I, I, P]),
    "fs2_intensity_head": (I, [P, I64, P, P, P, P, P, I, I, I, I, P, I, P]),
    "fs2_phoneme_average": (I, [P, I, I, P, P, I, I, P, P]),
    "fs2_rank_mixup_input": (I, [P, P, P, I, I, I, P, I, I, P]),
    "fs2_rank_pool": (I, [P, P, P, I, I, I, P, P, P]),
    "fs2_rank_loss_fwd": (I, [P, P, P, P, P, P, P, P, I, I, Fl, Fl, P, P]),
    "fs2_bucket_means": (I, [P, P, P, P, P, I, I, I, P, P]),
    "fs2_gelu_dropout_fwd": (I, [P, I64, I, P, I64, P, I64, I, I, Fl, U32, U32, I, P]),
    "fs2_gelu_dropout_bwd": (I, [P, I64, P, I64, P, I64, I, I, Fl, U32, U32, I, P]),
    "fs2_intensity_head_bwd": (I, [P, P, I64, P, P, I, P, P, I, I, I, I, P, I64, P, P, P, P, I,
                                   P]),
    "fs2_intensity_head_bwd_workspace_floats": (I64, [I, I, I, I]),
    "fs2_rank_pool_bwd": (I, [P, P, P, P, P, P, I, I, I, P, P, P]),
    "fs2_rank_loss_fwd_bwd": (I, [P, P, P, P, P, P, P, P, I, I, Fl, Fl, P, P, P, P, P, P]),
    "fs2_collate_phonemes": (I, [P, P, P, P, I, I, P, P, P, P]),
    "fs2_collate_frames": (I, [P, P, P, P, P, I, I, I, P, P, P, P, P, P]),
    "fs2_rank_collate": (I, [P, P, P, P, P, I, I, I, P, P, P, P]),
    "fs2_store_collate": (I, [P, P, P, P, I, I, I, I, I, P, P, P, P, P, P, P, P, P, P]),
    "fs2_vocoder_input": (I, [P, I, I, I, I, P, I, I, P]),
    "fs2_leaky_relu": (I, [P, P, I64, Fl, I, P]),
    "fs2_mean3_leaky_relu": (I, [P, P, P, P, I64, Fl, I, P]),
    "fs2_melspec": (I, [P, P, I, P, P, P, P, I, I, I, I, I, I, I, P, P, P, P]),
    "fs2_energy_minmax": (I, [P, P, I, I, P, P]),
    "fs2_prosody_track": (I, [P, I, P, P, P, P, P, I, I, I, I, P, P, P, P]),
    "fs2_prosody_stats": (I, [P, P, P, P, I, P, P]),
    "fs2_prosody_normalize": (I, [P, P, P, P, P, I, I, I, P, P, P, P]),
    "fs2_prosody_minmax": (I, [P, P, P, P, I, P, P]),
    "fs2_fill": (I, [P, I64, Fl, I, P]),
    "fs2_add": (I, [P, P, I64, Fl, I, P]),
    "fs2_cast": (I, [P, I, P, I, I64, P]),
    "fs2_set_dropout_seed": (I, [U32, P]),
    "fs2_version": (ctypes.c_char_p, []),
    "fs2_source_hash": (ctypes.c_char_p, []),
}

_lib = None


_CSRC = os.path.join(os.path.dirname(_HERE), "csrc")
_HEADER = os.path.join(os.path.dirname(os.path.dirname(_HERE)), "include", "fs2_hip.h")


# ... 76 lines not shown
```

fine-grained-emotional-control-of-tts_amd/fastspeech2/engine.py:

```python

import contextlib
import re

import torch

from . import _native as N
from . import lowering
from . import ops
from .attention import attention_bwd, attention_fwd, use_flash
from .lowering import BK, dgrad_split, eff_split, ps_plain_ok, round_up, wgrad_slices


class _Salt:
    def __init__(self):
        self.n = 0

    def __call__(self):
        self.n += 1
        return self.n


_NO_SIDE = N.exp_flag("FS2_NO_SIDE_STREAM")
_NO_AUX = N.exp_flag("FS2_NO_AUX_STREAM")
_SIDE_CTAS = 208


class FS2Engine:
    def __init__(self, model, act_dtype=torch.float32):
        self.m = model
        self.cfg = model.cfg
        self.adt = act_dtype
        self.dt = N.dtype_code(act_dtype)
        self.epc = ops.EPC[self.dt]
        N.load()
        model._ensure_packed()
        self.dev = model._flat.device
        self.params = dict(model.named_parameters())
        self.grads = dict(model._grad_views)
        self.pe_enc = model.sinusoidal_positional_embed_encoder.pe[0].float().contiguous()
        self.pe_dec = model.sinusoidal_positional_embed_decoder.pe[0].float().contiguous()
        self._ws = torch.empty(1 << 20, dtype=torch.float32, device=self.dev)
        self._ws_key = torch.cuda.current_stream(self.dev).cuda_stream
        self._ws_other = {}
        self._side = torch.cuda.Stream(self.dev) if (self.dt == N.BF16 and not _NO_SIDE) else None
        self._side_ctas = min(256, max(8, _SIDE_CTAS // 8 * 8)) if self._side is not None else 256
        self._aux = torch.cuda.Stream(self.dev) if (self._side is not None and not _NO_AUX) else None
        self.w = {}
        self._wspecs = self._weight_specs()
        self._fuse_pred_conv1()
        self._prepared_version = None
        self._wtable = None
        self.on_grads_ready = None
        self.timer = None
        self._km = {}
        self._offs = {}
        self._img = {}
        self._fimg = {}
        self.adam_split = None
        self._adam_late_done = False
        self.dp_late = None
        self.n_adam_late = 0
        self._adam_tabs = None
        self.skip_grad_tail = True
        self.check_grad_tail = False
        self.grad_tail_checked = []

    def _dec_halo(self):
        return sum((self._wspecs[f"decoder.layers.{i}.pos_ffn.{j}.conv.weight"][2] - 1) // 2
                   for i in range(self.cfg.dec_num_layers) for j in (0, 2))

    def _postnet_halo(self):
        return sum((kw - 1) // 2 for n, (_, _, kw) in self._wspecs.items()
                   if n.startswith("postnet."))

    def _tail_on(self):
        return self.skip_grad_tail or self.check_grad_tail

    def _km_offs(self, grad_end, P):
        ent = self._offs.get(id(grad_end))
        if ent is None or ent[0] is not grad_end or ent[1] != P:
            return None
        return ent[2]

    def _grad_end(self, mel_len, T, halo, P):
        end, offs = ops.grad_tail_bounds(mel_len.contiguous(), T, halo, P)
        self._offs[id(end)] = (end, P, offs)
        return end

    def _tail_bound(self, site, dy, B, T, grad_end, L=None):
        if grad_end is None:
            return None
        if self.check_grad_tail:
            L = L or T
            t = torch.arange(T, device=self.dev)[None, :] >= grad_end[:, None].long()
            tail = dy[:B * L].reshape(B, L, -1)[:, :T][t]
            nz = int((tail != 0).sum())
            assert nz == 0, f"{site}: {nz} non-zero gradient elements past grad_end"
            self.grad_tail_checked.append((site, int(tail.shape[0])))
        return grad_end if self.skip_grad_tail else None

    def _fwd_image(self, rows, tail, C):
        key = (rows, tail, C, self.adt)
        img = self._fimg.get(key)
        if img is None:
            img = self.empty(rows + tail, C)
            img[rows:].zero_()
            self._fimg[key] = img
        return img

    def _tic(self, tag):
        if tag and self.timer is not None:
            self.timer.start(tag)

    def _toc(self, tag):
        if tag and self.timer is not None:
            self.timer.stop(tag)

    @contextlib.contextmanager
    def _timed(self, kind, T):
        tag = self._dtag(kind, "", T)
        self._tic(tag)
        try:
            yield
        finally:
            self._toc(tag)

    def use_flash(self, T, dh):
        return use_flash(T, dh, self.dt)

    def ws(self, n):
        n = int(n)
        key = N.stream_ptr()
        buf = self._ws if key == self._ws_key else self._ws_other.get(key)
        if buf is None or buf.numel() < n:
            buf = torch.empty(max(int(n * 1.25) + 1024, 1 << 20), dtype=torch.float32,
                              device=self.dev)
            if key == self._ws_key:
                self._ws = buf
            else:
                self._ws_other[key] = buf
        return buf

    def _side_enter(self, *tensors):
        if self._side is None:
            return None
        main = torch.cuda.current_stream(self.dev)
        if self._aux is not None and main.cuda_stream == self._aux.cuda_stream:
            return None
        self._side.wait_stream(main)
        ctx = torch.cuda.stream(self._side)
        ctx.__enter__()
        return ctx, tensors

    def _side_exit(self, h):
        if h is None:
            return
        ctx, tensors = h
        ctx.__exit__(None, None, None)
        for t in tensors:
            if t is not None:
                t.record_stream(self._side)

    def _aux_fork(self, *tensors):
        main = torch.cuda.current_stream(self.dev)
        self._aux.wait_stream(main)
        for t in tensors:
            if t is not None:
                t.record_stream(self._aux)
        ctx = torch.cuda.stream(self._aux)
        ctx.__enter__()
        return ctx, main

    def _aux_exit(self, h):
        h[0].__exit__(None, None, None)

    def _aux_join(self, main, *tensors):
        main.wait_stream(self._aux)
        for t in tensors:
            if t is not None:
                t.record_stream(main)

# ... 149 lines not shown
        m = self.m
        if not self._adam_late_done:
            self.adamw_step(opt, *scal)
            return
        self._adam_late_done = False
        we, re_ = self._adam_tabs[0]
        torch.cuda.current_stream(self.dev).wait_stream(self._aux)
        ops.adamw_prep(we, re_, m._flat, m._gflat, opt.exp_avg, opt.exp_avg_sq, *scal, dt=self.dt)
        m.mark_params_updated()
        self._prepared_version = (m._param_version, m._flat._version)

    def _dtag(self, kind, wname, T):
        if self.timer is None or not getattr(self.timer, "detail", False):
            return None
        return f"{kind}:{re.sub(r'layers[.][0-9]+', 'layers.*', wname)}:T{T}"

    def _fwd(self, X, ldx, M, T, wname, out, ldo, **epi):
        O, C, KW = self._wspecs[wname]
        Wf, _ = self.w[wname]
        K = Wf.shape[1]
        ti = self._okc[wname] & lowering.W_TAP_INNER_FWD
        tag = self._dtag("fwd", wname, T)
        self._tic(tag)
        if isinstance(X, tuple):
            P = (KW - 1) // 2
            ops.gemm((M // T) * (T + 2 * P), O, K, X[0], C, Wf, K, out, ldo, dt=self.dt,
                     c_row=(T, -2 * P), a_kw=KW if ti else 0, **epi)
        else:
            if ti:
                raise ValueError(f"{wname}: its forward image is in the tap-inner order of the "
                                 "padded-image path, which this batch cannot take")
            ops.gemm(M, O, K, X, ldx, Wf, K, out, ldo, dt=self.dt,
                     conv=(1, T, KW, C) if KW > 1 else None, **epi)
        self._toc(tag)

    def _dgrad(self, dY, lddy, M, T, wname, out, ldo, n_out=None, **epi):
        tag = self._dtag("dgrad", wname, T)
        self._tic(tag)
        self._dgrad_impl(dY, lddy, M, T, wname, out, ldo, n_out, **epi)
        self._toc(tag)

    def _dy_image(self, key, B, T, P, F):
        L = T + 2 * P
        n = (B + 1) * L * F
        shape = (B, T, P, F)
        if torch.cuda.is_current_stream_capturing():
            buf = torch.empty(n, dtype=self.adt, device=self.dev)
            buf.view(B + 1, L, F)[:, T:].zero_()
        else:
            ent = self._img.get(key)
            if ent is None or ent[0] != shape:
                buf = ent[1] if ent is not None and ent[1].numel() >= n else \
                    torch.empty(n, dtype=self.adt, device=self.dev)
                buf[:n].view(B + 1, L, F)[:, T:].zero_()
                ent = self._img[key] = (shape, buf)
            buf = ent[1]
        img = buf[:n].view((B + 1) * L, F)[T:]
        return img, img[2 * P:]

    def _dgrad_impl(self, dY, lddy, M, T, wname, out, ldo, n_out=None, **epi):
        O, C, KW = self._wspecs[wname]
        _, Wb = self.w[wname]
        if KW == 1:
            ops.gemm(M, n_out or C, O, dY, lddy, Wb, O, out, ldo, dt=self.dt, **epi)
            return
        P = (KW - 1) // 2
        B = M // T
        Mp = B * (T + 2 * P)
        ti = isinstance(dY, tuple) and self._okc[wname] & lowering.W_TAP_INNER
        split = 1 if ti else lowering.dgrad_split(Mp, C, KW * O, self.dt)
        stride = Mp * C if split > 1 else 0
        Xpad = torch.empty(split, Mp, C, dtype=torch.float32, device=self.dev)
        if isinstance(dY, tuple):
            ops.gemm(Mp, C, KW * O, dY[0], O, Wb, KW * O, Xpad, C, dt=self.dt, c_fp32=1,
                     split_k=split, split_stride=stride, a_kw=KW if ti else 0)
        else:
            ops.gemm(Mp, C, KW * O, dY, lddy, Wb, KW * O, Xpad, C, dt=self.dt,
                     conv=(4, T, KW, O), c_fp32=1, split_k=split, split_stride=stride)
        ops.conv_fold(Xpad, B, T, P, C, out, ldo, dt=self.dt, nsplit=split, split_stride=Mp * C,
                      **epi)

    def _wgrad(self, dY, lddy, X, ldx, M, T, wname, n_cols=None, gemm_tag=None, bias=None,
               dy_img=None, grad_end=None):
        grad_end = self._tail_bound(wname, dY, M // T, T, grad_end,
                                    T + self._wspecs[wname][2] - 1 if dy_img is not None else None)
        h = self._side_enter(dY, X, dy_img, grad_end)
        tag = self._dtag("wgrad", wname, T)
        self._tic(tag)
        ctas = self._side_ctas if h is not None else 0
        done = self._wgrad_impl(dY, lddy, X, ldx, M, T, wname, n_cols, gemm_tag, bias, dy_img,
                                ctas, grad_end)
        self._toc(tag)
        if bias is not None and not done:
            O = self._wspecs[wname][0]
            ops.colsum(dY, lddy, M, O, self.grads[bias], dt=self.dt, ws=self.ws(ops.colsum_ws(M, O)))
        self._side_exit(h)

    def _km_image(self, key, C, ld):
        n = C * ld
        if torch.cuda.is_current_stream_capturing():
            return torch.zeros(n + 128, dtype=torch.bfloat16, device=self.dev)[64:64 + n]
        k = (key, C)
        ent = self._km.get(k)
        if ent is None or ent[1].numel() < n + 128:
            buf = torch.zeros(n + 128, dtype=torch.bfloat16, device=self.dev)
            self._km[k] = (ld, buf)
        elif ent[0] != ld:
            buf = ent[1]
            buf[64 + n:64 + n + 64].zero_()
            self._km[k] = (ld, buf)
        else:
            buf = ent[1]
        return buf[64:64 + n]

    def _wgrad_km(self, dY, lddy, X, ldx, M, T, wname, gemm_tag=None, bias=None, dy_img=None,
                  ctas=0, grad_end=None):
        O, C, KW = self._wspecs[wname]
        P = (KW - 1) // 2
        B = M // T
        p = lowering.wgrad_plan(O, C, KW, self.dt, M, T, lddy, ldx, None, ctas)
        Kp, S, stride = p.K, p.ns, p.stride
        dYT = self._km_image("dy", O, Kp)
        XT = self._km_image("x", C, Kp)
        ws = self.ws(max(ops.pad_transpose_ws(Kp, O), 1))
        colsum = self.grads[bias] if bias is not None else None
        keff, bk = None, {}
        offs = self._km_offs(grad_end, P) if grad_end is not None and Kp >= 128 else None
        if offs is not None:
            keff, bk = offs[B:B + 1], dict(offs=offs, ksplit=S)
        if dy_img is not None:
            ops.pad_transpose(dy_img[P:], lddy, B, T + 2 * P, O, 0, 0, dYT, Kp, Kp,
                              dt=self.dt, colsum=colsum, ws=ws, **bk)
        else:
            ops.pad_transpose(dY, lddy, B, T, O, P, 0, dYT, Kp, Kp, dt=self.dt, colsum=colsum,
                              ws=ws, **bk)
        ops.pad_transpose(X, ldx, B, T, C, P, 1, XT, Kp, Kp, dt=self.dt, **bk)
        ws = self.ws(p.ws_floats)
        self._tic(gemm_tag)
        ops.gemm(O, p.ldc, Kp, dYT, Kp, XT, Kp, ws, p.ldc, dt=self.dt, conv=(6, T, KW, C),
                 c_fp32=1, split_k=S, split_stride=stride if S > 1 else 0, max_ctas=ctas,
                 k_eff=keff)
        self._toc(gemm_tag)
        ops.sum_slices(ws, S, stride, stride, self.grads[wname], accumulate=p.accumulate)
        return True

    def _wgrad_impl(self, dY, lddy, X, ldx, M, T, wname, n_cols=None, gemm_tag=None, bias=None,
                    dy_img=None, ctas=0, grad_end=None):
        O, C, KW = self._wspecs[wname]
        if lowering.km_ok(O, C, KW, self.dt, T, n_cols, lddy, ldx):
            return self._wgrad_km(dY, lddy, X, ldx, M, T, wname, gemm_tag, bias, dy_img, ctas,
                                  grad_end)
        if dy_img is not None:
            raise RuntimeError(f"{wname}: a padded dY image needs the K-major weight gradient")
        p = lowering.wgrad_plan(O, C, KW, self.dt, M, T, lddy, ldx, n_cols, ctas)
        ns, stride = p.ns, p.stride
        atomic = p.path == "atomic"
        out = self.grads[wname] if atomic else self.ws(p.ws_floats)
        tag = gemm_tag if p.path == "slices" else None
        self._tic(tag)
        ops.gemm(O, n_cols or KW * C, p.K, dY, lddy, X, ldx, out, p.ldc, dt=self.dt, a_kmajor=0,
                 b_kmajor=0, conv=(3, T, KW, C) if KW > 1 else None, c_fp32=1, kvalid=M,
                 nvalid=p.ldc, accumulate=int(atomic), split_k=ns, split_stride=stride,
                 max_ctas=ctas)
        self._toc(tag)
        if p.path == "slices":
            ops.sum_slices(out, ns, stride, stride, self.grads[wname], accumulate=p.accumulate)
        elif p.path == "cols":
            tot = out[ns * stride:(ns + 1) * stride]
            ops.sum_slices(out, ns, stride, stride, tot, accumulate=p.accumulate)
            self.grads[wname].view(O, C).add_(tot.view(O, p.ldc)[:, :C])

    def _bias_grad(self, dY, lddy, M, n, gname):
        h = self._side_enter(dY)
        ops.colsum(dY, lddy, M, n, self.grads[gname], dt=self.dt, ws=self.ws(ops.colsum_ws(M, n)))
        self._side_exit(h)

    def _fft_fwd(self, X, B, T, key_pad, prefix, H, p_drop, seed, salt):
        D = self.cfg.enc_d_model
        M = B * T
        P = self.params
        ctx = {"X": X}
        QKV = self.empty(M, 3 * D)
        self._fwd(X, D, M, T, prefix + "self_att.att.in_proj_weight", QKV, 3 * D,
                  bias=P[prefix + "self_att.att.in_proj_bias"])
        Att = self.empty(M, D)
        s_att = salt()
        ctx.update(attention_fwd(QKV, key_pad, B, H, T, D, Att, dt=self.dt, dev=self.dev,
                                 mask_mode=1, p_drop=p_drop, seed=seed, salt=s_att,
                                 empty=self.empty, timed=self._timed("attn_fwd", T)),
                   key_pad=key_pad)
        Ao = self.empty(M, D)
        self._fwd(Att, D, M, T, prefix + "self_att.att.out_proj.weight", Ao, D,
                  bias=P[prefix + "self_att.att.out_proj.bias"])
        X1, s1 = self.empty(M, D), self.empty(M, D)
        mean1 = torch.empty(M, dtype=torch.float32, device=self.dev)
        rstd1 = torch.empty_like(mean1)
        s_r1 = salt()
        w1 = prefix + "pos_ffn.0.conv.weight"
        F, _, KW1 = self._wspecs[w1]
        P1 = (KW1 - 1) // 2
        img = self._fwd_image(B * (T + 2 * P1), 2 * P1, D) if lowering.fwd_padded(
            F, D, KW1, self.dt, M, T, self._okc[w1]) else None
        ops.ln_fwd(X, D, P[prefix + "norm1.norm.weight"], P[prefix + "norm1.norm.bias"], 1e-6, X1, D,
                   mean1, rstd1, M, D, dt=self.dt, seed=seed, r=Ao, ldr=D, p_r=p_drop, salt_r=s_r1,
                   s_out=s1, img=img, img_t=T, img_p=P1)
        del Ao
        Hc = self.empty(M, F)
        X1in = X1 if img is None else (img,)
        tag = "ffn_conv1_fwd." + prefix.split(".")[0]
        self._tic(tag)
        self._fwd(X1in, D, M, T, w1, Hc, F, bias=P[prefix + "pos_ffn.0.conv.bias"], relu=1)
        self._toc(tag)
        del X1in, img
        Y = self.empty(M, D)
        self._fwd(Hc, F, M, T, prefix + "pos_ffn.2.conv.weight", Y, D,
                  bias=P[prefix + "pos_ffn.2.conv.bias"])
        X2, s2 = self.empty(M, D), self.empty(M, D)
        mean2 = torch.empty(M, dtype=torch.float32, device=self.dev)
        rstd2 = torch.empty_like(mean2)
        s_r2 = salt()
        ops.ln_fwd(X1, D, P[prefix + "norm2.norm.weight"], P[prefix + "norm2.norm.bias"], 1e-6, X2, D,
                   mean2, rstd2, M, D, dt=self.dt, seed=seed, r=Y, ldr=D, p_r=p_drop, salt_r=s_r2,
                   s_out=s2)
        ctx.update(QKV=QKV, Att=Att, X1=X1, s1=s1, mean1=mean1, rstd1=rstd1, Hc=Hc, s2=s2,
                   mean2=mean2, rstd2=rstd2, s_att=s_att, s_r1=s_r1, s_r2=s_r2, F=F)
        return X2, ctx

    def _fft_bwd(self, dX2, ctx, B, T, prefix, H, p_drop, seed, grad_end=None):
        D = self.cfg.enc_d_model
        M = B * T
        F = ctx["F"]
        P, G = self.params, self.grads
        lnws = self.ws(ops.ln_ws(M, D))
        ds2, dY = self.empty(M, D), self.empty(M, D)
        ops.ln_bwd(dX2, D, ctx["s2"], D, ctx["mean2"], ctx["rstd2"], P[prefix + "norm2.norm.weight"],
                   P[prefix + "norm2.norm.bias"], ds2, D, M, D, dt=self.dt, ws=lnws, seed=seed,
                   dr=dY, p_r=p_drop, salt_r=ctx["s_r2"], dgamma=G[prefix + "norm2.norm.weight"],
                   dbeta=G[prefix + "norm2.norm.bias"], dcol=G[prefix + "pos_ffn.2.conv.bias"])
        w2 = prefix + "pos_ffn.2.conv.weight"
        w1 = prefix + "pos_ffn.0.conv.weight"
        pad = self._okc[w1] & lowering.W_REV
        if pad:
            refusal = lowering.dgrad_refusal(*self._wspecs[w1], B, T)
            if refusal:
                raise ValueError(f"{w1}: {refusal}")
            P1 = (self._wspecs[w1][2] - 1) // 2
            img, dHc = self._dy_image(prefix, B, T, P1, F)
            crow = {"c_row": (T, 2 * P1)}
        else:
            img, crow = None, {}
            dHc = self.empty(M, F)
        dX1 = self.empty(M, D)
        self._wgrad(dY, D, ctx["Hc"], F, M, T, w2)
        self._dgrad(dY, D, M, T, w2, dHc, F, gate=ctx["Hc"], ldg=F, **crow)
        self._wgrad(dHc, F, ctx["X1"], D, M, T, w1,
                    gemm_tag="ffn_conv1_wgrad." + prefix.split(".")[0],
                    bias=prefix + "pos_ffn.0.conv.bias", dy_img=img, grad_end=grad_end)
        self._dgrad((img,) if pad else dHc, F, M, T, w1, dX1, D, residual=ds2, ldr=D)
        del dY, dHc, ds2, img
        lnws = self.ws(ops.ln_ws(M, D))
        ds1, dAo = self.empty(M, D), self.empty(M, D)
        ops.ln_bwd(dX1, D, ctx["s1"], D, ctx["mean1"], ctx["rstd1"], P[prefix + "norm1.norm.weight"],
                   P[prefix + "norm1.norm.bias"], ds1, D, M, D, dt=self.dt, ws=lnws, seed=seed,
                   dr=dAo, p_r=p_drop, salt_r=ctx["s_r1"], dgamma=G[prefix + "norm1.norm.weight"],
                   dbeta=G[prefix + "norm1.norm.bias"],
                   dcol=G[prefix + "self_att.att.out_proj.bias"])
        del dX1
        wo = prefix + "self_att.att.out_proj.weight"
        dAtt = self.empty(M, D)
        self._wgrad(dAo, D, ctx["Att"], D, M, T, wo)
        self._dgrad(dAo, D, M, T, wo, dAtt, D)
        del dAo
        dQKV = self.empty(M, 3 * D)
        qb = self._tail_bound(prefix + "attn_bwd", dAtt, B, T, grad_end) if "lse" in ctx else None
        attention_bwd(ctx["QKV"], ctx["key_pad"], ctx["Att"], dAtt, ctx, B, H, T, D, dQKV,
                      dt=self.dt, dev=self.dev, mask_mode=1, p_drop=p_drop, seed=seed,
                      salt=ctx["s_att"], empty=self.empty, ws=self.ws, q_bound=qb,
                      timed=self._timed("attn_bwd", T))
        wi = prefix + "self_att.att.in_proj_weight"
        dX = self.empty(M, D)
        self._wgrad(dQKV, 3 * D, ctx["X"], D, M, T, wi)
        self._bias_grad(dQKV, 3 * D, M, 3 * D, prefix + "self_att.att.in_proj_bias")
        self._dgrad(dQKV, 3 * D, M, T, wi, dX, D, residual=ds1, ldr=D)
        return dX

    def _pred_fwd(self, Zin, keep, B, T, name, rate, p_drop, seed, salt, a1=None, lda1=None,
                  salts=None):
        D = self.cfg.enc_d_model
        M = B * T
        P = self.params
        c = {"Zin": Zin}
        if a1 is None:
            a1, lda1 = self.empty(M, D), D
            self._fwd(Zin, D, M, T, name + ".conv1.conv.weight", a1, D,
                      bias=P[name + ".conv1.conv.bias"], relu=1)
        v1 = self.empty(M, D)
        m1 = torch.empty(M, dtype=torch.float32, device=self.dev)
        r1 = torch.empty_like(m1)
        s1 = salts[0] if salts else salt()
        ops.ln_fwd(a1, lda1, P[name + ".ln1.norm.weight"], P[name + ".ln1.norm.bias"], 1e-5, v1, D, m1,
                   r1, M, D, dt=self.dt, seed=seed, p_o=p_drop, salt_o=s1, row_mask=keep)
        a2 = self.empty(M, D)
        self._fwd(v1, D, M, T, name + ".conv2.conv.weight", a2, D,
                  bias=P[name + ".conv2.conv.bias"], relu=1)
        v2 = self.empty(M, D)
        m2 = torch.empty(M, dtype=torch.float32, device=self.dev)
        r2 = torch.empty_like(m2)
        s2 = salts[1] if salts else salt()
        ops.ln_fwd(a2, D, P[name + ".ln2.norm.weight"], P[name + ".ln2.norm.bias"], 1e-5, v2, D, m2, r2,
                   M, D, dt=self.dt, seed=seed, p_o=p_drop, salt_o=s2, row_mask=keep)
        y = self.empty(B, T)
        ops.rowdot_fwd(v2, D, P[name + ".linear.w.weight"], P[name + ".linear.w.bias"], float(rate),
                       M, D, y, dt=self.dt)
        c.update(a1=a1, lda1=lda1, v1=v1, m1=m1, r1=r1, a2=a2, v2=v2, m2=m2, r2=r2, s1=s1, s2=s2,
                 rate=float(rate))
        return y, c

    def _pred_pair_fwd(self, Zin, keep, B, T, pitch_rate, p_drop, seed, salt):
        if self.PRED1 not in self._wspecs:
            pd, dctx = self._pred_fwd(Zin, keep, B, T, "durPred", 1.0, p_drop, seed, salt)
            pp, pctx = self._pred_fwd(Zin, keep, B, T, "pitchPred", pitch_rate, p_drop, seed, salt)
            return pd, dctx, pp, pctx
        D = self.cfg.enc_d_model
        M = B * T
        a1 = self.empty(M, 2 * D)
        self._fwd(Zin, D, M, T, self.PRED1, a1, 2 * D, bias=self.params[self.PRED1 + ".bias"],
                  relu=1)
        sd = (salt(), salt())
        sp = (salt(), salt())
        pd, dctx = self._pred_fwd(Zin, keep, B, T, "durPred", 1.0, p_drop, seed, salt,
                                  a1=a1[:, :D], lda1=2 * D, salts=sd)
        pp, pctx = self._pred_fwd(Zin, keep, B, T, "pitchPred", pitch_rate, p_drop, seed, salt,
                                  a1=a1[:, D:], lda1=2 * D, salts=sp)
        dctx["a1_pair"] = a1
        return pd, dctx, pp, pctx

    def _pred_pair_bwd(self, d_dur, dctx, d_pitch, pctx, keep, B, T, p_drop, seed, residual=None,
                       post_mask=False):
        if "a1_pair" not in dctx:
            dZa = self._pred_bwd(d_pitch, pctx, keep, B, T, "pitchPred", p_drop, seed,
                                 residual=residual)
            return self._pred_bwd(d_dur, dctx, keep, B, T, "durPred", p_drop, seed, residual=dZa,
                                  post_mask=post_mask)
        D = self.cfg.enc_d_model
        M = B * T
        da1 = self.empty(M, 2 * D)
        self._pred_bwd(d_pitch, pctx, keep, B, T, "pitchPred", p_drop, seed, da1=da1[:, D:])
        self._pred_bwd(d_dur, dctx, keep, B, T, "durPred", p_drop, seed, da1=da1[:, :D])
        dZ = self.empty(M, D)
        self._dgrad(da1, 2 * D, M, T, self.PRED1, dZ, D, row_scale=keep, residual=residual,
                    ldr=D if residual is not None else 0,
                    row_scale_post=keep if post_mask else None)
        self._wgrad(da1, 2 * D, dctx["Zin"], D, M, T, self.PRED1)
        return dZ

    def _pred_bwd(self, dy, c, keep, B, T, name, p_drop, seed, residual=None, post_mask=False,
                  da1=None):
        D = self.cfg.enc_d_model
        M = B * T
        P, G = self.params, self.grads
        dv2 = self.empty(M, D)
        nb = min(256, max(1, (M + 31) // 32))
        ops.rowdot_bwd(dy, c["v2"], D, P[name + ".linear.w.weight"], c["rate"], M, D, dv2,
                       G[name + ".linear.w.weight"], G[name + ".linear.w.bias"], dt=self.dt,
# ... 204 lines not shown
            durs, d_is_float = durations.contiguous(), 0
        else:
            durs = torch.clamp(torch.special.expm1(pd.float()), min=0).contiguous()
            d_is_float = 1
        mel_len = torch.empty(B, dtype=torch.int64, device=self.dev)
        cum = torch.empty(B, Tp, dtype=torch.int32, device=self.dev)
        if mel_len_max is None:
            ops.lr_index(durs, d_is_float, float(pace), B, Tp, 0, mel_len, cum, None)
            mel_lens_host = mel_len.cpu()
            Tm = int(mel_lens_host.max())
        else:
            Tm = int(mel_len_max)
            mel_lens_host = None
        frame_src = torch.empty(B, Tm, dtype=torch.int32, device=self.dev)
        ops.lr_index(durs, d_is_float, float(pace), B, Tp, Tm, mel_len, cum, frame_src)
        Mm = B * Tm
        S0 = self.empty(Mm, D)
        keep_m = torch.empty(Mm, dtype=torch.float32, device=self.dev)
        ops.lr_gather(Z3, frame_src, self.pe_dec, B, Tp, Tm, D, S0, keep_m, dt=self.dt)
        kp_dec = torch.empty(Mm, dtype=torch.uint8, device=self.dev)
        ops.keypad_from_lengths(mel_len, B, Tm, kp_dec)
        Xd = S0
        dec_ctx = []
        for i in range(c.dec_num_layers):
            Xd, lc = self._fft_fwd(Xd, B, Tm, kp_dec, f"decoder.layers.{i}.", H_d, pe_dec_p, seed, salt)
            dec_ctx.append(lc)
        Xo = self.empty(Mm, D)
        md = torch.empty(Mm, dtype=torch.float32, device=self.dev)
        rd = torch.empty_like(md)
        ops.ln_fwd(Xd, D, P["decoder.norm.norm.weight"], P["decoder.norm.norm.bias"], 1e-6, Xo, D, md,
                   rd, Mm, D, dt=self.dt)
        mel = self.empty(Mm, NM)
        self._fwd(Xo, D, Mm, Tm, "linear.w.weight", mel, NM, bias=P["linear.w.bias"],
                  row_scale=keep_m)
        post, pn_ctx = self._postnet_fwd(mel, B, Tm, pp_, seed, salt)
        if aux_h is not None:
            self._aux_join(aux_h[1], pd, pp, pe_, *[t for cc in (dctx, pctx, ectx)
                                                    for t in cc.values()
                                                    if isinstance(t, torch.Tensor)])
        ctx.update(keep_p=keep_p, enc_ctx=enc_ctx, Xenc_last=X, me=me, re=re_, cat=cat, ldc=ldc,
                   Z=Z, dctx=dctx, pctx=pctx, ectx=ectx, a_p=a_p, a_e=a_e, Z2m=Z2m, Tm=Tm,
                   cum=cum, keep_m=keep_m, dec_ctx=dec_ctx, Xdec_last=Xd, md=md, rd=rd, Xo=Xo,
                   pn_ctx=pn_ctx, p_enc=pe_enc_p, p_dec=pe_dec_p, p_var=pv, p_post=pp_,
                   mel_len=mel_len)
        out = (mel.view(B, Tm, NM), post.view(B, Tm, NM), pd.view(B, Tp), pp.view(B, Tp, 1),
               None if avg_p is None else avg_p.view(B, Tp, 1), pe_.view(B, Tp, 1),
               None if avg_e is None else avg_e.view(B, Tp, 1),
               mel_lens_host if mel_lens_host is not None else mel_len)
        return out, ctx

    def backward(self, ctx, d_mel, d_post, d_dur, d_pitch, d_energy):
        c = self.cfg
        D, H_e, H_d, NM = c.enc_d_model, c.enc_num_head, c.dec_num_head, c.n_mels
        B, Tp, Tm, seed = ctx["B"], ctx["Tp"], ctx["Tm"], ctx["seed"]
        Mp, Mm = B * Tp, B * Tm
        P, G = self.params, self.grads
        keep_p, keep_m = ctx["keep_p"], ctx["keep_m"]
        def notify(tag):
            if self.on_grads_ready is not None:
                self.on_grads_ready(tag, self.grad_streams())
                if (self.dp_late is not None and self.adam_split is not None
                        and not self._adam_late_done and self._aux is not None
                        and self._side is not None and self.dp_late[0]()):
                    self._adam_launch_late(self.dp_late[1])
        self._offs = {}
        d_mel = d_mel.reshape(Mm, NM).to(self.adt).contiguous()
        d_post = d_post.reshape(Mm, NM).to(self.adt).contiguous()
        d_pitch = d_pitch.reshape(Mp).to(self.adt).contiguous()
        d_dur = d_dur.reshape(Mp).to(self.adt).contiguous()
        aux_h, dZd, dZp, dZe = None, None, None, None
        d_energy = d_energy.reshape(Mp).to(self.adt).contiguous()
        if self._aux is not None:
            aux_h = self._aux_fork(d_pitch, d_dur, d_energy, keep_p)
            dZpd = self._pred_pair_bwd(d_dur, ctx["dctx"], d_pitch, ctx["pctx"], keep_p, B, Tp,
                                       ctx["p_var"], seed)
            dZe = self._pred_bwd(d_energy, ctx["ectx"], keep_p, B, Tp, "energyPred",
                                 ctx["p_var"], seed)
            self._aux_exit(aux_h)
        d_mel_total = d_mel.clone()
        ops.add(d_mel_total, d_post, Mm * NM, 1.0, dt=self.dt)
        dmel = self._postnet_bwd(d_post, d_mel_total, keep_m, ctx["pn_ctx"], B, Tm, ctx["p_post"],
                                 seed, ctx["mel_len"])
        notify("postnet")
        dXo = self.empty(Mm, D)
        self._dgrad(dmel, NM, Mm, Tm, "linear.w.weight", dXo, D)
        self._wgrad(dmel, NM, ctx["Xo"], D, Mm, Tm, "linear.w.weight")
        self._bias_grad(dmel, NM, Mm, NM, "linear.w.bias")
        dX = self.empty(Mm, D)
        ops.ln_bwd(dXo, D, ctx["Xdec_last"], D, ctx["md"], ctx["rd"], P["decoder.norm.norm.weight"],
                   P["decoder.norm.norm.bias"], dX, D, Mm, D, dt=self.dt, ws=self.ws(ops.ln_ws(Mm, D)),
                   dgamma=G["decoder.norm.norm.weight"], dbeta=G["decoder.norm.norm.bias"])
        notify("linear")
        dec_end = None
        if self._tail_on():
            P1 = (self._wspecs["decoder.layers.0.pos_ffn.0.conv.weight"][2] - 1) // 2
            dec_end = self._grad_end(ctx["mel_len"], Tm, self._dec_halo(), P1)
        for i in reversed(range(c.dec_num_layers)):
            dX = self._fft_bwd(dX, ctx["dec_ctx"][i], B, Tm, f"decoder.layers.{i}.", H_d,
                               ctx["p_dec"], seed, grad_end=dec_end)
            notify(f"decoder.layers.{i}")
        dZ3 = self.empty(Mp, D)
        ops.lr_scatter(dX, ctx["cum"], keep_m, B, Tp, Tm, D, dZ3, dt=self.dt)
        def wg_side(fn, *tensors):
            h = self._side_enter(*tensors)
            fn()
            self._side_exit(h)
        kwe = c.energy_pred_kernel_size
        wg_side(lambda: ops.embed1d_bwd(dZ3, ctx["a_e"], B, Tp, D, kwe, G["energyEmbed.conv.weight"],
                                        G["energyEmbed.conv.bias"], dt=self.dt,
                                        ws=self.ws(128 * (kwe + 1) * D)), dZ3, ctx["a_e"])
        if dZe is not None:
            self._aux_join(aux_h[1], dZpd, dZe)
            dZ2 = dZe
            ops.add(dZ2, dZ3, Mp * D, 1.0, dt=self.dt)
        else:
            dZ2 = self._pred_bwd(d_energy, ctx["ectx"], keep_p, B, Tp, "energyPred", ctx["p_var"],
                                 seed, residual=dZ3)
        kwp = c.pitch_pred_kernel_size
        wg_side(lambda: ops.embed1d_bwd(dZ2, ctx["a_p"], B, Tp, D, kwp, G["pitchEmbed.conv.weight"],
                                        G["pitchEmbed.conv.bias"], dt=self.dt,
                                        ws=self.ws(128 * (kwp + 1) * D)), dZ2, ctx["a_p"])
        if aux_h is not None:
            self._aux_join(aux_h[1], dZpd)
            dZ = dZpd
            ops.add3_mask_rows(dZ, dZ2, None, D, keep_p, Mp, D, dt=self.dt)
        else:
            dZ = self._pred_pair_bwd(d_dur, ctx["dctx"], d_pitch, ctx["pctx"], keep_p, B, Tp,
                                     ctx["p_var"], seed, residual=dZ2, post_mask=True)
        notify("variance")
        if (self.adam_split is not None and self._aux is not None and self._side is not None
                and self.on_grads_ready is None
                and not torch.cuda.is_current_stream_capturing()):
            self._adam_launch_late()
        ldc = ctx["ldc"]
        dcat = self.empty(Mp, 2 * D)
        self._dgrad(dZ, D, Mp, Tp, "concat_proj.w.weight", dcat, 2 * D, n_out=2 * D)
        self._wgrad(dZ, D, ctx["cat"], ldc, Mp, Tp, "concat_proj.w.weight", n_cols=ldc)
        wg_side(lambda: ops.concat_bwd_spk(dcat, 2 * D, ctx["speakers"], B, Tp, D, c.n_speakers,
                                           G["speaker_emb.Embedding.weight"], dt=self.dt,
                                           ws=self.ws(B * D)), dcat, ctx["speakers"])
        dXl = self.empty(Mp, D)
        ops.ln_bwd(dcat, 2 * D, ctx["Xenc_last"], D, ctx["me"], ctx["re"], P["encoder.norm.norm.weight"],
                   P["encoder.norm.norm.bias"], dXl, D, Mp, D, dt=self.dt,
                   ws=self.ws(ops.ln_ws(Mp, D)), row_mask=keep_p,
                   dgamma=G["encoder.norm.norm.weight"], dbeta=G["encoder.norm.norm.bias"])
        notify("conditioning")
        dX = dXl
        for i in reversed(range(c.enc_num_layers)):
            dX = self._fft_bwd(dX, ctx["enc_ctx"][i], B, Tp, f"encoder.layers.{i}.", H_e,
                               ctx["p_enc"], seed)
            notify(f"encoder.layers.{i}")
        ops.embed_bwd(ctx["tokens"], dX, keep_p, Mp, D, c.n_char,
                      G["encPreNet.token_embedding.Embedding.weight"], dt=self.dt,
                      ws=self.ws(ops.embed_bwd_ws(D, c.n_char)))
        self.side_join()
        notify("prenet")
```

fine-grained-emotional-control-of-tts_amd/fastspeech2/ops.py:

```python

import collections
import ctypes
import os
import sys

import torch

from . import _native as N
from .lowering import EPC, round_up


def _p(x):
    if x is None:
        return None
    if isinstance(x, int):
        return x
    return x.data_ptr()


def _s():
    return N.stream_ptr()


def _chk(rc, name):
    if rc != 0:
        raise RuntimeError(f"{name} returned {rc}")


_TRACE = collections.Counter() if os.environ.get("FS2_GEMM_TRACE") else None

GemmPlan = collections.namedtuple(
    "GemmPlan", "kernel grid block tiles_m tiles_n split_k k_per_split vec_ok accumulate")


def _plan(d):
    i = N.GemmPlanInfo()
    _chk(N.lib().fs2_gemm_plan(ctypes.byref(d), ctypes.byref(i)), "fs2_gemm_plan")
    return GemmPlan(i.kernel.decode(), tuple(i.grid), i.block, i.tiles_m, i.tiles_n, i.split_k,
                    i.k_per_split, i.vec_ok, i.accumulate)


def _trace(d):
    f = sys._getframe(2)
    while f is not None and os.path.basename(f.f_code.co_filename) == "ops.py":
        f = f.f_back
    site = f"{f.f_code.co_name}:{f.f_lineno}" if f is not None else "?"
    flags = "".join(k for k, v in (("a", not d.a_kmajor), ("b", not d.b_kmajor), ("f", d.c_fp32),
                                   ("B", d.bias), ("r", d.relu), ("g", d.gate), ("R", d.residual),
                                   ("s", d.row_scale), ("S", d.row_scale_post),
                                   ("+", d.accumulate), ("c", d.c_row_t)) if v)
    pl = _plan(d)
    _TRACE[(d.M, d.N, d.K, d.conv_mode, d.split_k, d.batch, flags, pl.kernel, pl.grid, site)] += 1


def _trace_dump():
    for k, n in sorted(_TRACE.items(), key=lambda x: -x[0][0] * x[0][1] * x[0][2] * x[1]):
        M, N_, K, cm, sk, b, fl, kern, grid, site = k
        print(f"gemm {n:4d}x M {M:6d} N {N_:5d} K {K:6d} conv {cm} split {sk} batch {b:4d} "
              f"[{fl}] {kern} grid {grid[0]}x{grid[2]} {site}", file=sys.stderr)


if _TRACE is not None:
    import atexit
    atexit.register(_trace_dump)


def gemm(M, N_, K, A, lda, B, ldb, C, ldc, *, dt, a_kmajor=1, b_kmajor=1, conv=None, c_fp32=0,
         c_conv_kw=0, bias=None, relu=0, gate=None, ldg=0, row_scale=None, residual=None, ldr=0,
         row_scale_post=None, accumulate=0, split_k=1, split_stride=0, kvalid=0, mvalid=0,
         nvalid=0, batch=1, batch_div=1, strides=None, conv_dil=1, c_row=None, max_ctas=0,
         a_kw=0, k_eff=None, plan=False):
    d = N.GemmDesc()
    d.k_eff = _p(k_eff)
    d.conv_dil = conv_dil
    d.a_kw = a_kw
    d.max_ctas = max_ctas
    if c_row is not None:
        d.c_row_t, d.c_row_pad = c_row
    d.M, d.N, d.K, d.kvalid, d.mvalid, d.nvalid, d.dtype = M, N_, K, kvalid, mvalid, nvalid, dt
    d.A, d.lda, d.a_kmajor = _p(A), lda, a_kmajor
    d.B, d.ldb, d.b_kmajor = _p(B), ldb, b_kmajor
    if conv is not None:
        d.conv_mode, d.conv_t, d.conv_kw, d.conv_c = conv
    d.C, d.ldc, d.c_fp32, d.c_conv_kw = _p(C), ldc, c_fp32, c_conv_kw
    d.bias, d.relu = _p(bias), relu
    d.gate, d.ldg = _p(gate), ldg
    d.row_scale = _p(row_scale)
    d.residual, d.ldr = _p(residual), ldr
    d.row_scale_post = _p(row_scale_post)
    d.accumulate, d.split_k, d.split_stride = accumulate, split_k, split_stride
    d.batch, d.batch_div = batch, batch_div
    if strides is not None:
        (d.sA1, d.sA2, d.sB1, d.sB2, d.sC1, d.sC2, d.sR1, d.sR2) = strides
    if plan:
        return _plan(d)
    if _TRACE is not None:
        _trace(d)
    _chk(N.lib().fs2_gemm(ctypes.byref(d), _s()), "fs2_gemm")


def gemm_plan(*args, **kw):
    return gemm(*args, plan=True, **kw)


def conv_fold(Xpad, B, T, P, C, out, ldo, *, dt, residual=None, ldr=0, row_scale=None,
              row_scale_post=None, nsplit=1, split_stride=0):
    _chk(N.lib().fs2_conv_fold(_p(Xpad), nsplit, split_stride, B, T, P, C, _p(out), ldo,
                               _p(residual), ldr,
                               _p(row_scale), _p(row_scale_post), dt, _s()), "fs2_conv_fold")


def grad_tail_bounds(mel_len, T, halo, P):
    B = mel_len.numel()
    assert mel_len.dtype == torch.int64 and mel_len.is_contiguous()
    end = torch.empty(B, dtype=torch.int32, device=mel_len.device)
    offs = torch.empty(round_up(B + 1, 16) + 16, dtype=torch.int32, device=mel_len.device)
    _chk(N.lib().fs2_grad_tail_bounds(_p(mel_len), B, T, halo, P, _p(end), _p(offs), offs.numel(),
                                      _s()), "fs2_grad_tail_bounds")
    return end, offs


_TRI = {}


def km_offsets(grad_end, T, P):
    B = grad_end.numel()
    key = (B, grad_end.device)
    tri = _TRI.get(key)
    if tri is None:
        tri = torch.ones(B, B, dtype=torch.int32, device=grad_end.device).tril()
        if not torch.cuda.is_current_stream_capturing():
            _TRI[key] = tri
    offs = torch.full((round_up(B + 1, 16) + 16,), 2 ** 31 - 1, dtype=torch.int32,
                      device=grad_end.device)
    offs[0] = 0
    Tp = T + 2 * P
    start = torch.arange(B, dtype=torch.int32, device=grad_end.device) * Tp
    drop = ((start + Tp) // 64 - (start + grad_end + 2 * P + 63) // 64).clamp(min=0)
    offs[1:B + 1] = (tri * (Tp - 64 * drop)[None, :]).sum(1, dtype=torch.int32)
    return offs


def pad_transpose(X, ldx, B, T, C, P, reflect, out, ldo, ncols, *, dt, colsum=None, ws=None,
                  offs=None, ksplit=1):
    if offs is not None:
        assert offs.dtype == torch.int32 and offs.numel() >= round_up(B + 1, 16) + 16
        _chk(N.lib().fs2_pad_transpose_bounded(_p(X), ldx, B, T, C, P, reflect, _p(out), ldo,
                                               ncols, _p(colsum), _p(ws), _p(offs), ksplit, dt,
                                               _s()), "fs2_pad_transpose_bounded")
        return
    _chk(N.lib().fs2_pad_transpose(_p(X), ldx, B, T, C, P, reflect, _p(out), ldo, ncols,
                                   _p(colsum), _p(ws), dt, _s()), "fs2_pad_transpose")


def pad_rows(X, ldx, B, T, C, P, reflect, tail, out, ldo, *, dt):
    _chk(N.lib().fs2_pad_rows(_p(X), ldx, B, T, C, P, reflect, tail, _p(out), ldo, dt, _s()),
         "fs2_pad_rows")


def pad_transpose_ws(ncols, C):
    return -(-ncols // 64) * C


def sum_slices(ws, nslices, stride, n, out, accumulate=1):
    _chk(N.lib().fs2_sum_slices(_p(ws), nslices, stride, n, _p(out), accumulate, _s()),
         "fs2_sum_slices")


def colsum(X, ldx, M, N_, out, *, dt, ws, accumulate=1):
    _chk(N.lib().fs2_colsum(_p(X), ldx, M, N_, dt, _p(out), accumulate, _p(ws), _s()), "fs2_colsum")


def colsum_ws(M, N_):
    return N.lib().fs2_colsum_workspace_floats(M, N_)


def ln_fwd(x, ldx, gamma, beta, eps, y, ldy, mean, rstd, M, D, *, dt, seed=0, r=None, ldr=0,
           p_r=0.0, salt_r=0, s_out=None, do_tanh=0, p_o=0.0, salt_o=0, row_mask=None,
           post_add=None, ldp=0, img=None, img_t=0, img_p=0):
    _chk(N.lib().fs2_ln_fwd(_p(x), ldx, _p(r), ldr, p_r, salt_r, _p(s_out), _p(gamma), _p(beta),
                            eps, do_tanh, p_o, salt_o, _p(row_mask), _p(post_add), ldp, _p(y), ldy,
                            _p(mean), _p(rstd), M, D, dt, seed & 0xffffffff, _p(img), img_t, img_p,
                            _s()), "fs2_ln_fwd")


def ln_bwd(dy, lddy, s, lds, mean, rstd, gamma, beta, ds, ldds, M, D, *, dt, ws, seed=0,
           do_tanh=0, p_o=0.0, salt_o=0, row_mask=None, relu_gate_in=0, dr=None, p_r=0.0,
           salt_r=0, dgamma=None, dbeta=None, dcol=None):
    _chk(N.lib().fs2_ln_bwd(_p(dy), lddy, _p(s), lds, _p(mean), _p(rstd), _p(gamma), _p(beta),
                            do_tanh, p_o, salt_o, _p(row_mask), relu_gate_in, _p(ds), ldds, _p(dr),
                            p_r, salt_r, _p(dgamma), _p(dbeta), _p(dcol), M, D, dt,
                            seed & 0xffffffff,
                            _p(ws), _s()), "fs2_ln_bwd")


def ln_ws(M, D):
    return N.lib().fs2_ln_workspace_floats(M, D)


def attn_supported(T, dh, dt):
    return bool(N.lib().fs2_attn_supported(T, dh, dt))


def attn_fwd(qkv, ldq, key_pad, B, H, T, dh, scale, p_drop, seed, salt, out, ldo, lse, *, dt,
# ... 353 lines not shown
```

include/fs2_hip.h:

```cpp
#ifndef FS2_HIP_H
#define FS2_HIP_H

#include <stdint.h>

#ifdef __cplusplus
extern "C" {
#endif

#define FS2_F32 0
#define FS2_BF16 1

#define FS2_EINVAL (-1)
#define FS2_EALIGN (-2)

typedef struct fs2_gemm_desc {
  int M, N, K;
  int kvalid;
  int mvalid, nvalid;
  int dtype;
  const void* A; int64_t lda; int a_kmajor;
  const void* B; int64_t ldb; int b_kmajor;
  int conv_mode, conv_t, conv_kw, conv_c;
  void* C; int64_t ldc; int c_fp32;
  int c_conv_kw;
  const float* bias;
  int relu;
  const void* gate; int64_t ldg;
  const float* row_scale;
  const void* residual; int64_t ldr;
  const float* row_scale_post;
  int accumulate;
  int split_k;
  int64_t split_stride;
  int batch, batch_div;
  int64_t sA1, sA2, sB1, sB2, sC1, sC2, sR1, sR2;
  int conv_dil;
  int c_row_t, c_row_pad;
  int max_ctas;
  int a_kw;
  const int32_t* k_eff;
} fs2_gemm_desc;

int fs2_gemm(const fs2_gemm_desc* d, void* stream);

typedef struct fs2_gemm_plan_info {
  char kernel[64];
  int grid[3];
  int block;
  int tiles_m, tiles_n;
  int split_k, k_per_split;
  int vec_ok, accumulate;
} fs2_gemm_plan_info;

int fs2_gemm_plan(const fs2_gemm_desc* d, fs2_gemm_plan_info* out);

int fs2_conv_fold(const float* Xpad, int nsplit, int64_t split_stride, int B, int T, int P,
                  int C, void* out, int64_t ldo, const void* residual, int64_t ldr,
                  const float* row_scale, const float* row_scale_post, int dtype, void* stream);

int fs2_pad_transpose(const void* X, int64_t ldx, int B, int T, int C, int P, int reflect,
                      void* out, int64_t ldo, int ncols, float* colsum, float* workspace,
                      int dtype, void* stream);
int fs2_pad_transpose_bounded(const void* X, int64_t ldx, int B, int T, int C, int P, int reflect,
                              void* out, int64_t ldo, int ncols, float* colsum, float* workspace,
                              const int32_t* offs, int ksplit, int dtype, void* stream);

int fs2_grad_tail_bounds(const int64_t* len, int B, int T, int halo, int P, int32_t* end,
                         int32_t* offs, int noffs, void* stream);

int fs2_sum_slices(const float* ws, int nslices, int64_t stride, int64_t n, float* out,
                   int accumulate, void* stream);

int fs2_pad_rows(const void* X, int64_t ldx, int B, int T, int C, int P, int reflect, int tail,
                 void* out, int64_t ldo, int dtype, void* stream);

int fs2_colsum(const void* X, int64_t ldx, int M, int N, int dtype, float* out, int accumulate,
               float* workspace, void* stream);
int64_t fs2_colsum_workspace_floats(int M, int N);

int fs2_ln_fwd(const void* x, int64_t ldx, const void* r, int64_t ldr, float p_r, uint32_t salt_r,
               void* s_out, const float* gamma, const float* beta, float eps, int do_tanh,
               float p_o, uint32_t salt_o, const float* row_mask, const void* post_add,
               int64_t ldp, void* y, int64_t ldy, float* mean, float* rstd, int M, int D,
               int dtype, uint32_t seed, void* img, int img_t, int img_p, void* stream);

int fs2_ln_bwd(const void* dy, int64_t lddy, const void* s, int64_t lds, const float* mean,
               const float* rstd, const float* gamma, const float* beta, int do_tanh, float p_o,
               uint32_t salt_o, const float* row_mask, int relu_gate_in, void* ds, int64_t ldds,
               void* dr, float p_r, uint32_t salt_r, float* dgamma, float* dbeta, float* dcol,
               int M, int D,
               int dtype, uint32_t seed, float* workspace, void* stream);
int64_t fs2_ln_workspace_floats(int M, int D);

int fs2_softmax_fwd(const float* S, const uint8_t* key_pad, int mask_mode, int B, int H, int Tq,
                    int Tk, int ldt, float scale, float p_drop, uint32_t seed, uint32_t salt,
                    void* P, void* Pd, int dtype, void* stream);
int fs2_softmax_bwd(const float* dPd, const void* P, int B, int H, int Tq, int Tk, int ldt,
                    float scale, float p_drop, uint32_t seed, uint32_t salt, void* dS, int dtype,
                    void* stream);

int fs2_attn_supported(int T, int dh, int dtype);
int fs2_attn_fwd(const void* qkv, int64_t ldq, const uint8_t* key_pad, int mask_mode, int B,
                 int H, int T, int dh, float scale, float p_drop, uint32_t seed, uint32_t salt,
                 void* out, int64_t ldo, float* lse, int dtype, void* stream);
int fs2_attn_bwd(const void* qkv, int64_t ldq, const uint8_t* key_pad, int mask_mode,
                 const void* out,
                 int64_t ldo, const void* dout, int64_t lddo, const float* lse, int B, int H,
                 int T, int dh, float scale, float p_drop, uint32_t seed, uint32_t salt,
                 void* dqkv, int64_t lddq, float* workspace, int dtype, void* stream);
int fs2_attn_bwd_bounded(const void* qkv, int64_t ldq, const uint8_t* key_pad, int mask_mode,
                         const void* out, int64_t ldo, const void* dout, int64_t lddo,
                         const float* lse, int B, int H, int T, int dh, float scale,
                         float p_drop, uint32_t seed, uint32_t salt, void* dqkv, int64_t lddq,
                         float* workspace, const int32_t* q_bound, int dtype, void* stream);
int64_t fs2_attn_workspace_floats(int B, int H, int T);

int fs2_embed_fwd(const int64_t* tokens, const float* table, const float* pe, int pad_idx,
                  int B, int T, int D, void* X, float* keep, int dtype, void* stream);
int fs2_embed_bwd(const int64_t* tokens, const void* dX, const float* keep, int M, int D,
                  int V, float* dtable, float* workspace, int dtype, void* stream);
int64_t fs2_embed_bwd_workspace_floats(int D, int V);

int fs2_keypad_from_tokens(const int64_t* tokens, int pad_idx, int M, uint8_t* key_pad,
                           void* stream);
int fs2_keypad_from_lengths(const int64_t* lens, int B, int T, uint8_t* key_pad, float* keep,
                            void* stream);

int fs2_concat_fwd(const void* feats, const float* spk_table, const int64_t* spk,
                   const float* intensity, int B, int T, int D, int E, void* cat, int ldc,
                   int dtype, void* stream);
int fs2_concat_bwd_spk(const void* dcat, int ldc, const int64_t* spk, int B, int T, int D,
                       int n_spk, float* dspk, int dtype, float* workspace ,
                       void* stream);

int fs2_mask_rows(void* X, int64_t ldx, const float* keep, int M, int D, int dtype, void* stream);
int fs2_add3_mask_rows(void* X, const void* Y, const void* Z, int64_t ld, const float* keep,
                       int M, int D, int dtype, void* stream);

int fs2_rowdot_fwd(const void* u, int64_t ldu, const float* w, const float* b, float scale, int M,
                   int D, void* y, int dtype, void* stream);
int fs2_rowdot_bwd(const void* dy, const void* u, int64_t ldu, const float* w, float scale, int M,
                   int D, void* du, float* dw, float* db, int dtype, float* workspace,
                   void* stream);

int fs2_avg_over_durations(const float* values, int Tm_in, const int64_t* durs, int B, int Tp,
                           float* avg, float* workspace, void* stream);
int64_t fs2_avg_workspace_floats(int B, int Tm_in);

int fs2_embed1d_fwd(const void* base, const float* a, const float* W, const float* bias, int B,
                    int T, int D, int KW, void* out, int dtype, void* stream);
int fs2_embed1d_bwd(const void* dout, const float* a, int B, int T, int D, int KW, float* dW,
                    float* dbias, int dtype, float* workspace, void* stream);
// ... 148 lines not shown
```

Measured before the change: 1.516 million mel-frames/s.

## Skip dead padded K-tiles in weight-gradient GEMMs via a live-tile list

Adds a kernel that builds a compacted list of 64-row K tiles holding live (non-padded) gradient rows, taken from the per-sample grad_end bounds. The mn-major bf16 weight-gradient GEMM paths now iterate only over the listed tiles instead of the whole K range. This applies to 1x1 projections (FFN conv2, attention out/in proj, final linear). The aim is to avoid loading and multiplying padding rows whose gradients are zero. It costs one extra small kernel launch per decoder backward and an indirect tile lookup in the GEMM pipeline prologue and loop.

```diff
diff --git a/fine-grained-emotional-control-of-tts_amd/csrc/gemm.hip b/fine-grained-emotional-control-of-tts_amd/csrc/gemm.hip
--- a/fine-grained-emotional-control-of-tts_amd/csrc/gemm.hip
+++ b/fine-grained-emotional-control-of-tts_amd/csrc/gemm.hip
@@ -42,6 +42,18 @@
   int a_kw;
   const int32_t* k_eff;
 };
+
+typedef const __attribute__((address_space(4))) int32_t* ktl_ptr;
+__device__ __forceinline__ int ktl_rank(const int32_t* l, int t, int nk_all) {
+  return min(max(((ktl_ptr)l)[3 + 2 * min(max(t, 0), nk_all + 8)], 0), nk_all);
+}
+__device__ __forceinline__ int ktl_raw(const int32_t* l, int i, int nk_all) {
+  return ((ktl_ptr)l)[2 + 2 * min(i, nk_all + 8)];
+}
+__device__ __forceinline__ int ktl_clamp(int v, int nk_all) { return min(max(v, 0), nk_all - 1); }
+__device__ __forceinline__ int ktl_tile(const int32_t* l, int i, int nk_all) {
+  return ktl_clamp(ktl_raw(l, i, nk_all), nk_all);
+}
 
 __device__ __forceinline__ u32x4 add_bf16x8(u32x4 a, u32x4 b) {
   u32x4 r;
@@ -361,6 +373,15 @@
   const char* Ab = p.A + (zb * p.sA1 + zh * p.sA2) * ES;
   const char* Bb = p.B + (zb * p.sB1 + zh * p.sB2) * ES;
   const int kvalid = p.kvalid;
+  constexpr bool KL = sizeof(T) == 2 && !AK && !BKM && GA && GB;
+  const int32_t* const kl = KL ? p.k_eff : nullptr;
+  const int nk_all = (p.K + Cfg<T>::BK - 1) / Cfg<T>::BK;
+  int lt0 = 0, lt1 = 0;
+  if (KL && kl) {
+    lt0 = ktl_rank(kl, kbeg / Cfg<T>::BK, nk_all);
+    lt1 = ktl_rank(kl, (kend + Cfg<T>::BK - 1) / Cfg<T>::BK, nk_all);
+    if (lt1 <= lt0 && p.split_k > 1 && p.split_stride == 0) return;
+  }
 
   int rb[4] = {0, 0, 0, 0}, rt[4] = {0, 0, 0, 0};
   const int amode = (p.conv_mode == 1 || p.conv_mode == 2 || p.conv_mode == 4 || p.conv_mode == 5) ? p.conv_mode : 0;
@@ -409,16 +430,19 @@
     if constexpr (!GB) { if constexpr (BKM) store_kmajor<T>(lb, stB); else store_mnmajor<T>(lb, stB); }
   };
 
-  const int nk = (kend > kbeg) ? (kend - kbeg + BK - 1) / BK : 0;
+  const int nk = (KL && kl) ? max(lt1 - lt0, 0) : (kend > kbeg) ? (kend - kbeg + BK - 1) / BK : 0;
+  auto tile_k = [&](int kt) {
+    return (KL && kl) ? ktl_tile(kl, lt0 + kt, nk_all) * BK : kbeg + kt * BK;
+  };
   if (nk > 0) {
-    load_tiles(kbeg, 0);
+    load_tiles(tile_k(0), 0);
     store_tiles(0);
   }
   __syncthreads();
 
   for (int kt = 0; kt < nk; ++kt) {
     const int stage = kt & 1;
-    if (kt + 1 < nk) load_tiles(kbeg + (kt + 1) * BK, stage ^ 1);
+    if (kt + 1 < nk) load_tiles(tile_k(kt + 1), stage ^ 1);
     const char* la = smem + stage * 2 * TILE_BYTES;
     const char* lb = la + TILE_BYTES;
     if constexpr (ES == 2) {
@@ -744,6 +768,12 @@
     kt0 = blockIdx.z * kps;
     kt1 = min(nk_all, kt0 + kps);
   }
+  constexpr bool KL = !AK && !BKM && CM == 0 && B3 == 0;
+  const int32_t* const kl = KL ? p.k_eff : nullptr;
+  const int lt0 = (KL && kl) ? __builtin_amdgcn_readfirstlane(ktl_rank(kl, kt0, nk_all)) : kt0;
+  const int nk = (KL && kl) ? __builtin_amdgcn_readfirstlane(ktl_rank(kl, kt1, nk_all)) - lt0
+                            : kt1 - kt0;
+  if (KL && kl && nk <= 0 && p.split_k > 1 && p.split_stride == 0) return;
   const bool bconv3 = B3 >= 0 ? B3 == 1 : p.conv_mode == 3;
   const bool tap_uniform = CM > 0 ? true : (CM == 0 ? false : amode && (p.conv_c % 64) == 0);
   const int rpu = amode == 4 ? p.conv_t + 2 * p.conv_p : p.conv_t;
@@ -901,16 +931,18 @@
 #pragma unroll
     for (int j = 0; j < 4; ++j) acc[i][j] = f32x4{0.f, 0.f, 0.f, 0.f};
 
-  const int nk = kt1 - kt0;
-  if (nk > 0) issue(kt0, 0);
-  if (nk > 1) issue(kt0 + 1, 1);
+  auto ptile = [&](int l) { return (KL && kl) ? ktl_tile(kl, l, nk_all) : l; };
+  if (nk > 0) issue(ptile(lt0), 0);
+  if (nk > 1) issue(ptile(lt0 + 1), 1);
+  int pt = (KL && kl) ? ktl_raw(kl, lt0 + 2, nk_all) : 0;
   for (int it = 0; it < nk; ++it) {
     if (it + 1 < nk) asm volatile("s_waitcnt vmcnt(6)" ::: "memory");
     else asm volatile("s_waitcnt vmcnt(0)" ::: "memory");
     asm volatile("s_waitcnt lgkmcnt(0)" ::: "memory");
     __builtin_amdgcn_s_barrier();
     __builtin_amdgcn_sched_barrier(0);
-    if (it + 2 < nk) issue(kt0 + it + 2, (it + 2) % 3);
+    if (it + 2 < nk) issue((KL && kl) ? ktl_clamp(pt, nk_all) : kt0 + it + 2, (it + 2) % 3);
+    if (KL && kl) pt = ktl_raw(kl, lt0 + it + 3, nk_all);
     const char* la = smem + (it % 3) * BIG_STAGE;
     const char* lb = la + BIG_A;
     bf16x8 af[2][4], bfr[2][4];
@@ -1007,6 +1039,12 @@
     kt0 = blockIdx.z * kps;
     kt1 = min(nk_all, kt0 + kps);
   }
+  constexpr bool KL = !AK && !BKM && CM == 0 && B3 == 0;
+  const int32_t* const kl = KL ? p.k_eff : nullptr;
+  const int lt0 = (KL && kl) ? __builtin_amdgcn_readfirstlane(ktl_rank(kl, kt0, nk_all)) : kt0;
+  const int nk = (KL && kl) ? __builtin_amdgcn_readfirstlane(ktl_rank(kl, kt1, nk_all)) - lt0
+                            : kt1 - kt0;
+  if (KL && kl && nk <= 0 && p.split_k > 1 && p.split_stride == 0) return;
   const bool bconv3 = B3 >= 0 ? B3 == 1 : p.conv_mode == 3;
   const bool tap_uniform = CM > 0 ? true : (CM == 0 ? false : amode && (p.conv_c % 32) == 0);
   const int rpu = amode == 4 ? p.conv_t + 2 * p.conv_p : p.conv_t;
@@ -1167,8 +1205,8 @@
       }
     }
   };
-  auto issue = [&](int it, int reg) {
-    const int k0 = (kt0 + it) * 64 + (reg >> 1) * 32;
+  auto issue = [&](int it, int ktp, int reg) {
+    const int k0 = ktp * 64 + (reg >> 1) * 32;
     char* dst = smem + (it & 1) * G4_SLOT + reg * G4_REG;
     if ((reg & 1) == 0) issueA(dst, k0);
     else issueB(dst, k0);
@@ -1180,12 +1218,15 @@
 #pragma unroll
     for (int j = 0; j < 4; ++j) acc[i][j] = f32x4{0.f, 0.f, 0.f, 0.f};
 
-  const int nk = kt1 - kt0;
+  auto praw = [&](int l) { return (KL && kl) ? ktl_raw(kl, l, nk_all) : l; };
+  auto pclamp = [&](int v) { return (KL && kl) ? ktl_clamp(v, nk_all) : v; };
+  int p1 = praw(lt0 + 1), p2 = praw(lt0 + 2);
   if (nk > 0) {
-    issue(0, 1); issue(0, 0); issue(0, 3); issue(0, 2);
+    const int p0 = pclamp(praw(lt0));
+    issue(0, p0, 1); issue(0, p0, 0); issue(0, p0, 3); issue(0, p0, 2);
   }
   if (nk > 1) {
-    issue(1, 1); issue(1, 0);
+    issue(1, pclamp(p1), 1); issue(1, pclamp(p1), 0);
     asm volatile("s_waitcnt vmcnt(8)" ::: "memory");
   } else {
     asm volatile("s_waitcnt vmcnt(4)" ::: "memory");
@@ -1202,6 +1243,7 @@
   bf16x8 af[4], bfr[4];
   for (int it = 0; it < nk; ++it) {
     const bool more = it + 1 < nk;
+    const int p3 = (KL && kl) ? praw(lt0 + it + 3) : 0;
 #pragma unroll
     for (int ph = 0; ph < 4; ++ph) {
       const int s = ph >> 1, mq = ph & 1;
@@ -1218,7 +1260,10 @@
         af[i] = AK ? g4_frag_k(rA, wr * 128 + mq * 64 + i * 16 + (lane & 15), lane >> 4)
                    : frag_bf16_mnmajor_asm<512>(rA, wr * 128 + mq * 64 + i * 16, 0, lane);
       const bool iss = !noissue && (ph < 2 ? more : it + 2 < nk);
-      if (iss) issue(ph < 2 ? it + 1 : it + 2, 3 - ph);
+      if (iss) {
+        const int rel = ph < 2 ? it + 1 : it + 2;
+        issue(rel, (KL && kl) ? pclamp(ph < 2 ? p1 : p2) : kt0 + rel, 3 - ph);
+      }
       if (grp == 1 && (ph & 1) && !nowait && !noissue) {
         if (iss) {
           asm volatile("s_waitcnt vmcnt(8)" ::: "memory");
@@ -1253,6 +1298,7 @@
       __builtin_amdgcn_s_barrier();
       __builtin_amdgcn_sched_barrier(0);
     }
+    if (KL && kl) { p1 = p2; p2 = p3; }
   }
   if (stag && wr == 0) __builtin_amdgcn_s_barrier();
   asm volatile("s_waitcnt vmcnt(0) lgkmcnt(0)" ::: "memory");
@@ -2476,8 +2522,11 @@
   p.mvalid = d->mvalid > 0 ? min(d->mvalid, d->M) : d->M;
   p.nvalid = d->nvalid > 0 ? min(d->nvalid, d->N) : d->N;
   p.A = (const char*)d->A; p.lda = d->lda; p.B = (const char*)d->B; p.ldb = d->ldb;
-  p.conv_mode = d->conv_mode; p.conv_t = d->conv_t; p.conv_kw = d->conv_kw; p.conv_c = d->conv_c;
-  p.conv_p = d->conv_kw > 0 ? (d->conv_kw - 1) / 2 : 0;
+  const bool klist = d->conv_mode == 8;
+  if (!klist) {
+    p.conv_mode = d->conv_mode; p.conv_t = d->conv_t; p.conv_kw = d->conv_kw; p.conv_c = d->conv_c;
+    p.conv_p = d->conv_kw > 0 ? (d->conv_kw - 1) / 2 : 0;
+  }
   p.conv_dil = d->conv_dil > 1 ? d->conv_dil : 1;
   p.C = (char*)d->C; p.ldc = d->ldc; p.c_fp32 = d->c_fp32; p.c_conv_kw = d->c_conv_kw;
   p.bias = d->bias; p.relu = d->relu;
@@ -2499,8 +2548,10 @@
   p.max_ctas = d->max_ctas > 0 && d->max_ctas < 256 ? max(8, d->max_ctas / 8 * 8) : 256;
   p.a_kw = d->a_kw > 0 ? d->a_kw : 0;
   p.k_eff = d->k_eff;
-  if (p.k_eff && (d->conv_mode != 6 || p.K < 128)) return FS2_EINVAL;
-  if (p.a_kw && (d->dtype != FS2_BF16 || !d->a_kmajor || !d->b_kmajor || d->conv_mode ||
+  if (klist && (!p.k_eff || d->dtype != FS2_BF16 || d->a_kmajor || d->b_kmajor || batch > 1))
+    return FS2_EINVAL;
+  if (p.k_eff && !klist && (d->conv_mode != 6 || p.K < 128)) return FS2_EINVAL;
+  if (p.a_kw && (d->dtype != FS2_BF16 || !d->a_kmajor || !d->b_kmajor || p.conv_mode ||
                  batch > 1 || p.split_k > 1 || p.lda % 64 ||
                  (long)p.a_kw * p.lda != p.K))
     return FS2_EINVAL;
diff --git a/fine-grained-emotional-control-of-tts_amd/csrc/norm.hip b/fine-grained-emotional-control-of-tts_amd/csrc/norm.hip
--- a/fine-grained-emotional-control-of-tts_amd/csrc/norm.hip
+++ b/fine-grained-emotional-control-of-tts_amd/csrc/norm.hip
@@ -919,6 +919,35 @@
   }
   if (offs)
     for (int i = B + 1 + lane; i < noffs; i += 64) offs[i] = 0x7fffffff;
+}
+
+__global__ void __launch_bounds__(64) live_tiles_kernel(const int32_t* end, int B, int T,
+                                                        int32_t* tiles, int npairs) {
+  const int lane = threadIdx.x;
+  const long rows = (long)B * T;
+  const long nt = (rows + 63) / 64;
+  int n = 0;
+  for (long i0 = 0; i0 < nt; i0 += 64) {
+    const long i = i0 + lane;
+    bool live = false;
+    if (i < nt) {
+      const long r0 = i * 64, r1 = min(r0 + 64, rows);
+      const int b1 = (int)((r1 - 1) / T);
+      for (int b = (int)(r0 / T); b <= b1 && !live; ++b) {
+        const long u0 = (long)b * T;
+        const int e = min(max(end[b], 0), T);
+        live = max(r0, u0) < min(r1, u0 + e);
+      }
+    }
+    const unsigned long long m = __ballot(live);
+    const int rank = n + __popcll(m & ((1ull << lane) - 1));
+    if (i < nt) tiles[3 + 2 * i] = rank;
+    if (live) tiles[2 + 2 * rank] = (int32_t)i;
+    n += __popcll(m);
+  }
+  if (lane == 0) { tiles[0] = n; tiles[1] = (int32_t)nt; }
+  for (int j = n + lane; j < npairs; j += 64) tiles[2 + 2 * j] = 0;
+  for (int i = (int)nt + lane; i < npairs; i += 64) tiles[3 + 2 * i] = n;
 }
 
 __global__ void __launch_bounds__(256) pad_rows_kernel(const bf16* X, long ldx, int B, int T,
@@ -1182,6 +1211,18 @@
   return 0;
 }
 
+extern "C" int fs2_live_tiles(const int32_t* end, int B, int T, int32_t* tiles, int ntiles,
+                              void* stream) {
+  if (B <= 0) return 0;
+  if (!end || !tiles || T <= 0 || (long)B * T >= 0x7fffffffL ||
+      ntiles < 2 * (((long)B * T + 63) / 64 + 10) + 2)
+    return FS2_EINVAL;
+  hipLaunchKernelGGL(live_tiles_kernel, dim3(1), dim3(64), 0, (hipStream_t)stream, end, B, T,
+                     tiles, (ntiles - 2) / 2);
+  FS2_CHECK_LAUNCH();
+  return 0;
+}
+
 extern "C" int fs2_pad_rows(const void* X, int64_t ldx, int B, int T, int C, int P, int reflect,
                             int tail, void* out, int64_t ldo, int dtype, void* stream) {
   if (B <= 0 || T <= 0 || C <= 0) return 0;
diff --git a/fine-grained-emotional-control-of-tts_amd/fastspeech2/_native.py b/fine-grained-emotional-control-of-tts_amd/fastspeech2/_native.py
--- a/fine-grained-emotional-control-of-tts_amd/fastspeech2/_native.py
+++ b/fine-grained-emotional-control-of-tts_amd/fastspeech2/_native.py
@@ -108,6 +108,7 @@
     "fs2_pad_transpose": (I, [P, I64, I, I, I, I, I, P, I64, I, P, P, I, P]),
     "fs2_pad_transpose_bounded": (I, [P, I64, I, I, I, I, I, P, I64, I, P, P, P, I, I, P]),
     "fs2_grad_tail_bounds": (I, [P, I, I, I, I, P, P, I, P]),
+    "fs2_live_tiles": (I, [P, I, I, P, I, P]),
     "fs2_pad_rows": (I, [P, I64, I, I, I, I, I, I, P, I64, I, P]),
     "fs2_ln_fwd": (I, [P, I64, P, I64, Fl, U32, P, P, P, Fl, I, Fl, U32, P, P, I64, P, I64, P, P,
                        I, I, I, U32, P, I, I, P]),
diff --git a/fine-grained-emotional-control-of-tts_amd/fastspeech2/engine.py b/fine-grained-emotional-control-of-tts_amd/fastspeech2/engine.py
--- a/fine-grained-emotional-control-of-tts_amd/fastspeech2/engine.py
+++ b/fine-grained-emotional-control-of-tts_amd/fastspeech2/engine.py
@@ -64,6 +64,7 @@
         self.skip_grad_tail = True
         self.check_grad_tail = False
         self.grad_tail_checked = []
+        self.grad_tail_checked_tm = []
 
     def _dec_halo(self):
         return sum((self._wspecs[f"decoder.layers.{i}.pos_ffn.{j}.conv.weight"][2] - 1) // 2
@@ -82,12 +83,19 @@
             return None
         return ent[2]
 
-    def _grad_end(self, mel_len, T, halo, P):
+    def _k_tiles(self, grad_end):
+        ent = self._offs.get(id(grad_end))
+        if ent is None or ent[0] is not grad_end:
+            return None
+        return ent[3]
+
+    def _grad_end(self, mel_len, T, halo, P, tiles=False):
         end, offs = ops.grad_tail_bounds(mel_len.contiguous(), T, halo, P)
-        self._offs[id(end)] = (end, P, offs)
+        kt = ops.live_tiles(end, T) if tiles and self.dt == N.BF16 and self.skip_grad_tail else None
+        self._offs[id(end)] = (end, P, offs, kt)
         return end
 
-    def _tail_bound(self, site, dy, B, T, grad_end, L=None):
+    def _tail_bound(self, site, dy, B, T, grad_end, L=None, log=None):
         if grad_end is None:
             return None
         if self.check_grad_tail:
@@ -96,7 +104,7 @@
             tail = dy[:B * L].reshape(B, L, -1)[:, :T][t]
             nz = int((tail != 0).sum())
             assert nz == 0, f"{site}: {nz} non-zero gradient elements past grad_end"
-            self.grad_tail_checked.append((site, int(tail.shape[0])))
+            (self.grad_tail_checked if log is None else log).append((site, int(tail.shape[0])))
         return grad_end if self.skip_grad_tail else None
 
     def _fwd_image(self, rows, tail, C):
@@ -412,8 +420,10 @@
 
     def _wgrad(self, dY, lddy, X, ldx, M, T, wname, n_cols=None, gemm_tag=None, bias=None,
                dy_img=None, grad_end=None):
+        KW = self._wspecs[wname][2]
         grad_end = self._tail_bound(wname, dY, M // T, T, grad_end,
-                                    T + self._wspecs[wname][2] - 1 if dy_img is not None else None)
+                                    T + KW - 1 if dy_img is not None else None,
+                                    log=self.grad_tail_checked_tm if KW == 1 else None)
         h = self._side_enter(dY, X, dy_img, grad_end)
         tag = self._dtag("wgrad", wname, T)
         self._tic(tag)
@@ -487,11 +497,17 @@
         atomic = p.path == "atomic"
         out = self.grads[wname] if atomic else self.ws(p.ws_floats)
         tag = gemm_tag if p.path == "slices" else None
+        kt = {}
+        if grad_end is not None and KW == 1 and self.dt == N.BF16 and \
+                p.path in ("atomic", "slices"):
+            tiles = self._k_tiles(grad_end)
+            if tiles is not None:
+                kt = {"k_tiles": tiles}
         self._tic(tag)
         ops.gemm(O, n_cols or KW * C, p.K, dY, lddy, X, ldx, out, p.ldc, dt=self.dt, a_kmajor=0,
                  b_kmajor=0, conv=(3, T, KW, C) if KW > 1 else None, c_fp32=1, kvalid=M,
                  nvalid=p.ldc, accumulate=int(atomic), split_k=ns, split_stride=stride,
-                 max_ctas=ctas)
+                 max_ctas=ctas, **kt)
         self._toc(tag)
         if p.path == "slices":
             ops.sum_slices(out, ns, stride, stride, self.grads[wname], accumulate=p.accumulate)
@@ -581,7 +597,7 @@
             img, crow = None, {}
             dHc = self.empty(M, F)
         dX1 = self.empty(M, D)
-        self._wgrad(dY, D, ctx["Hc"], F, M, T, w2)
+        self._wgrad(dY, D, ctx["Hc"], F, M, T, w2, grad_end=grad_end)
         self._dgrad(dY, D, M, T, w2, dHc, F, gate=ctx["Hc"], ldg=F, **crow)
         self._wgrad(dHc, F, ctx["X1"], D, M, T, w1,
                     gemm_tag="ffn_conv1_wgrad." + prefix.split(".")[0],
@@ -598,7 +614,7 @@
         del dX1
         wo = prefix + "self_att.att.out_proj.weight"
         dAtt = self.empty(M, D)
-        self._wgrad(dAo, D, ctx["Att"], D, M, T, wo)
+        self._wgrad(dAo, D, ctx["Att"], D, M, T, wo, grad_end=grad_end)
         self._dgrad(dAo, D, M, T, wo, dAtt, D)
         del dAo
         dQKV = self.empty(M, 3 * D)
@@ -609,7 +625,7 @@
                       timed=self._timed("attn_bwd", T))
         wi = prefix + "self_att.att.in_proj_weight"
         dX = self.empty(M, D)
-        self._wgrad(dQKV, 3 * D, ctx["X"], D, M, T, wi)
+        self._wgrad(dQKV, 3 * D, ctx["X"], D, M, T, wi, grad_end=grad_end)
         self._bias_grad(dQKV, 3 * D, M, 3 * D, prefix + "self_att.att.in_proj_bias")
         self._dgrad(dQKV, 3 * D, M, T, wi, dX, D, residual=ds1, ldr=D)
         return dX
@@ -980,19 +996,19 @@
         dmel = self._postnet_bwd(d_post, d_mel_total, keep_m, ctx["pn_ctx"], B, Tm, ctx["p_post"],
                                  seed, ctx["mel_len"])
         notify("postnet")
+        dec_end = None
+        if self._tail_on():
+            P1 = (self._wspecs["decoder.layers.0.pos_ffn.0.conv.weight"][2] - 1) // 2
+            dec_end = self._grad_end(ctx["mel_len"], Tm, self._dec_halo(), P1, tiles=True)
         dXo = self.empty(Mm, D)
         self._dgrad(dmel, NM, Mm, Tm, "linear.w.weight", dXo, D)
-        self._wgrad(dmel, NM, ctx["Xo"], D, Mm, Tm, "linear.w.weight")
+        self._wgrad(dmel, NM, ctx["Xo"], D, Mm, Tm, "linear.w.weight", grad_end=dec_end)
         self._bias_grad(dmel, NM, Mm, NM, "linear.w.bias")
         dX = self.empty(Mm, D)
         ops.ln_bwd(dXo, D, ctx["Xdec_last"], D, ctx["md"], ctx["rd"], P["decoder.norm.norm.weight"],
                    P["decoder.norm.norm.bias"], dX, D, Mm, D, dt=self.dt, ws=self.ws(ops.ln_ws(Mm, D)),
                    dgamma=G["decoder.norm.norm.weight"], dbeta=G["decoder.norm.norm.bias"])
         notify("linear")
-        dec_end = None
-        if self._tail_on():
-            P1 = (self._wspecs["decoder.layers.0.pos_ffn.0.conv.weight"][2] - 1) // 2
-            dec_end = self._grad_end(ctx["mel_len"], Tm, self._dec_halo(), P1)
         for i in reversed(range(c.dec_num_layers)):
             dX = self._fft_bwd(dX, ctx["dec_ctx"][i], B, Tm, f"decoder.layers.{i}.", H_d,
                                ctx["p_dec"], seed, grad_end=dec_end)
diff --git a/fine-grained-emotional-control-of-tts_amd/fastspeech2/ops.py b/fine-grained-emotional-control-of-tts_amd/fastspeech2/ops.py
--- a/fine-grained-emotional-control-of-tts_amd/fastspeech2/ops.py
+++ b/fine-grained-emotional-control-of-tts_amd/fastspeech2/ops.py
@@ -69,9 +69,12 @@
          c_conv_kw=0, bias=None, relu=0, gate=None, ldg=0, row_scale=None, residual=None, ldr=0,
          row_scale_post=None, accumulate=0, split_k=1, split_stride=0, kvalid=0, mvalid=0,
          nvalid=0, batch=1, batch_div=1, strides=None, conv_dil=1, c_row=None, max_ctas=0,
-         a_kw=0, k_eff=None, plan=False):
+         a_kw=0, k_eff=None, k_tiles=None, plan=False):
     d = N.GemmDesc()
     d.k_eff = _p(k_eff)
+    if k_tiles is not None:
+        assert conv is None and k_eff is None
+        conv, d.k_eff = (8, 0, 0, 0), _p(k_tiles)
     d.conv_dil = conv_dil
     d.a_kw = a_kw
     d.max_ctas = max_ctas
@@ -120,6 +123,16 @@
     return end, offs
 
 
+def live_tiles(grad_end, T):
+    B = grad_end.numel()
+    assert grad_end.dtype == torch.int32 and grad_end.is_contiguous()
+    tiles = torch.empty(2 * (-(-B * T // 64) + 10) + 2, dtype=torch.int32,
+                        device=grad_end.device)
+    _chk(N.lib().fs2_live_tiles(_p(grad_end), B, T, _p(tiles), tiles.numel(), _s()),
+         "fs2_live_tiles")
+    return tiles
+
+
 _TRI = {}
 
 
diff --git a/include/fs2_hip.h b/include/fs2_hip.h
--- a/include/fs2_hip.h
+++ b/include/fs2_hip.h
@@ -68,6 +68,8 @@
 int fs2_grad_tail_bounds(const int64_t* len, int B, int T, int halo, int P, int32_t* end,
                          int32_t* offs, int noffs, void* stream);
 
+int fs2_live_tiles(const int32_t* end, int B, int T, int32_t* tiles, int ntiles, void* stream);
+
 int fs2_sum_slices(const float* ws, int nslices, int64_t stride, int64_t n, float* out,
                    int accumulate, void* stream);
 
```

New measurement: 1.523 million mel-frames/s (median of 6 runs). No clear change (+0.4%).
